# exfinen/zk-toolkit

Hardware: AMD Instinct MI355X
Metric: G1 MSM scalar-muls/sec at 2^20 bases per GPU (BLS12-381) (higher is better)
Workload: dtype u32 limbs (384-bit Montgomery integer)

## Files before the change

### zk-toolkit_amd/csrc/zkt_api.cpp

```cpp
#include <hip/hip_runtime.h>
#include <mutex>
#include <vector>
#include <cstring>
#include <cstdio>
#include <cstdlib>
#include "../../include/zkt.h"
#include "zkt_internal.h"
#include "zkt_constants.h"
#include "host_abi.h"
static_assert(ZKT_G1_PARTIAL_WORDS == 3 * zkt::FqC::N && ZKT_G2_PARTIAL_WORDS == 6 * zkt::FqC::N && ZKT_SECP_PARTIAL_WORDS == 3 * zkt::SpC::N,
              "include/zkt.h partial sizes follow the internal limb layout");

using namespace zkt;

namespace {

struct Ctx {
  bool ready = false;
  int device = -1;
  hipStream_t stream = nullptr;
  unsigned long long* d_err = nullptr;
  uint8_t* arena = nullptr; size_t arena_bytes = 0;
  uint32_t* d_small = nullptr;
  std::mutex mu;
};
Ctx g;
thread_local size_t t_err_index = 0;
thread_local float t_kernel_ms = 0.f;
thread_local const char* t_kernel_name = "";

int ensure_ready() {
  if (!g.ready) return ZKT_ERR_DEVICE;
  return hipSetDevice(g.device) == hipSuccess ? ZKT_OK : ZKT_ERR_DEVICE;
}

int arena_reserve(size_t bytes) {
  if (bytes <= g.arena_bytes) return ZKT_OK;
  if (g.arena) { HIPCHK(hipFree(g.arena)); g.arena = nullptr; g.arena_bytes = 0; }
  size_t want = bytes + (bytes >> 2) + (1 << 20);
  HIPCHK(hipMalloc((void**)&g.arena, want));
  g.arena_bytes = want;
  return ZKT_OK;
}
struct Carver {
  uint8_t* p; size_t off = 0;
  explicit Carver(uint8_t* base) : p(base) {}
  template <class T> T* take(size_t bytes) { off = (off + 255) & ~size_t(255); T* r = (T*)(p + off); off += bytes; return r; }
};
size_t padded(size_t b) { return (b + 255) & ~size_t(255); }

int reset_err(hipStream_t s) {
  unsigned long long v = NO_ERR;
  HIPCHK(hipMemcpyAsync(g.d_err, &v, sizeof(v), hipMemcpyHostToDevice, s));
  return ZKT_OK;
}
int fetch_err(hipStream_t s, int code_if_set) {
  unsigned long long v = NO_ERR;
  HIPCHK(hipMemcpyAsync(&v, g.d_err, sizeof(v), hipMemcpyDeviceToHost, s));
  HIPCHK(hipStreamSynchronize(s));
  if (v != NO_ERR) { t_err_index = (size_t)v; return code_if_set; }
  return ZKT_OK;
}

template <class Launch>
int staged_raw(const void* a, size_t a_total, const void* b, size_t b_total, void* out, size_t out_total, int err_code, Launch launch) {
  if (ensure_ready() != ZKT_OK) return ZKT_ERR_DEVICE;
  if (!a || !out || (b_total && !b)) return ZKT_ERR_SHAPE;
  std::lock_guard<std::mutex> lk(g.mu);
  HIPCHK(hipSetDevice(g.device));
  int rc = arena_reserve(padded(a_total) + padded(b_total) + padded(out_total) + 1024);
  if (rc) return rc;
  Carver cv(g.arena);
  uint32_t* da = cv.take<uint32_t>(a_total);
  uint32_t* db = b_total ? cv.take<uint32_t>(b_total) : nullptr;
  uint32_t* dout = cv.take<uint32_t>(out_total);
  HIPCHK(hipMemcpyAsync(da, a, a_total, hipMemcpyHostToDevice, g.stream));
  if (db) HIPCHK(hipMemcpyAsync(db, b, b_total, hipMemcpyHostToDevice, g.stream));
  if ((rc = reset_err(g.stream))) return rc;
  HIPCHK(launch(da, db, dout, g.stream));
  HIPCHK(hipMemcpyAsync(out, dout, out_total, hipMemcpyDeviceToHost, g.stream));
  return fetch_err(g.stream, err_code);
}
template <class Launch>
int staged(const void* a, size_t a_bytes, const void* b, size_t b_bytes, void* out, size_t out_bytes, size_t n, int err_code, Launch launch) {
  if (ensure_ready() != ZKT_OK) return ZKT_ERR_DEVICE;
  if (n == 0) return ZKT_OK;
  return staged_raw(a, a_bytes * n, b, b_bytes * n, out, out_bytes * n, err_code, launch);
}

size_t field_bytes(int field) { return field == F_FQ ? 48 : 32; }
int fp_batch(int field, int op, const uint64_t* a, const uint64_t* b, uint64_t* out, size_t n) {
  const size_t w = field_bytes(field);
  const bool binary = op == OP_ADD || op == OP_SUB || op == OP_MUL;
  return staged(a, w, binary ? b : nullptr, binary ? w : 0, out, w, n, ZKT_ERR_INV_ZERO,
                [&](uint32_t* da, uint32_t* db, uint32_t* dout, hipStream_t s) { return launch_fp_op(field, op, da, db, dout, n, g.d_err, s); });
}
int fp_pow_batch(int field, const uint64_t* a, const uint64_t* exps, size_t exp_limbs, int exp_shared, uint64_t* out, size_t n) {
  if (exp_limbs == 0 || exp_limbs > 64) return ZKT_ERR_SHAPE;
  if (n == 0) return ensure_ready();
  const size_t w = field_bytes(field);
  return staged_raw(a, w * n, exps, exp_limbs * 8 * (exp_shared ? 1 : n), out, w * n, ZKT_ERR_SHAPE,
                    [&](uint32_t* da, uint32_t* db, uint32_t* dout, hipStream_t s) { return launch_fp_pow(field, da, db, (int)exp_limbs * 2, exp_shared != 0, dout, n, s); });
}
int fp_pow_seq(int field, const uint64_t* base, size_t n, uint64_t* out, bool repeat) {
  if (n == 0) return ensure_ready();
  const size_t w = field_bytes(field);
  return staged_raw(base, w, nullptr, 0, out, w * n, ZKT_ERR_SHAPE,
                    [&](uint32_t* da, uint32_t*, uint32_t* dout, hipStream_t s) { return launch_fp_pow_seq(field, da, dout, n, repeat, s); });
}
int fp_sum(int field, const uint64_t* a, size_t n, uint64_t* out) {
  if (ensure_ready() != ZKT_OK) return ZKT_ERR_DEVICE;
  if (n == 0 || !a || !out) return ZKT_ERR_SHAPE;
  const size_t w = field_bytes(field);
  std::lock_guard<std::mutex> lk(g.mu);
  HIPCHK(hipSetDevice(g.device));
  int rc = arena_reserve(padded(w * n) + padded(w * (1 + fp_sum_scratch_elems())) + 1024);
  if (rc) return rc;
  Carver cv(g.arena);
  uint32_t* da = cv.take<uint32_t>(w * n); uint32_t* dout = cv.take<uint32_t>(w * (1 + fp_sum_scratch_elems()));
  HIPCHK(hipMemcpyAsync(da, a, w * n, hipMemcpyHostToDevice, g.stream));
  HIPCHK(launch_fp_sum(field, da, n, dout, dout + w / 4, g.stream));
  HIPCHK(hipMemcpyAsync(out, dout, w, hipMemcpyDeviceToHost, g.stream));
  HIPCHK(hipStreamSynchronize(g.stream));
  return ZKT_OK;
}
int fp_scale(int field, const uint64_t* a, const uint64_t* k, uint64_t* out, size_t n) {
  if (n == 0) return ZKT_ERR_SHAPE;
  const size_t w = field_bytes(field);
  return staged_raw(a, w * n, k, w, out, w * n, ZKT_ERR_SHAPE,
                    [&](uint32_t* da, uint32_t* db, uint32_t* dout, hipStream_t s) { return launch_fp_scale(field, da, db, dout, n, s); });
}
int tower_batch(int deg, int op, const uint64_t* a, const uint64_t* b, uint64_t* out, size_t n) {
  const size_t w = (size_t)deg * 48;
  const bool binary = op == T_ADD || op == T_SUB || op == T_MUL;
  return staged(a, w, binary ? b : nullptr, binary ? w : 0, out, w, n, ZKT_ERR_INV_ZERO,
                [&](uint32_t* da, uint32_t* db, uint32_t* dout, hipStream_t s) { return launch_tower_op(deg, op, da, db, dout, n, g.d_err, s); });
}

}

static constexpr int MSM_SLOTS = 8;
struct MsmSlot {
  hipEvent_t e_in = nullptr, e_sorted = nullptr, e_acc0 = nullptr, e_acc1 = nullptr, e_done = nullptr;
  void* workspace = nullptr;
  uint32_t* d_result_jac = nullptr;
  uint32_t* d_out_abi = nullptr;
  uint8_t* h_out = nullptr;
  bool busy = false;
  static constexpr int NGRAPH = 4;
  hipGraphExec_t gexec[NGRAPH] = {}; const void* gkey[NGRAPH] = {}; unsigned gnext = 0; bool timed = false;
};
struct zkt_bases_impl {
  size_t n = 0;
  int grp = G_G1;
  MsmPlan plan{};
  uint32_t* table = nullptr;
  uint8_t* inf = nullptr;
  static constexpr int GROUP_TAILS = 4;
  static constexpr int NTAIL = 8;
  hipStream_t s_sort = nullptr, s_acc = nullptr, s_tail[NTAIL] = {};
  bool own_streams = true, acc_owned = false, grouped = false; int tail_base = 0, tail_span = 0;
  MsmSlot slot[MSM_SLOTS];
  std::mutex mu;
};
struct zkt_g1_bases : zkt_bases_impl {};
struct zkt_g2_bases : zkt_bases_impl {};
struct zkt_secp_bases : zkt_bases_impl {};
static size_t grp_coord_bytes(int grp) { return 4 * (grp == G_G1 ? zkt::FqC::N : grp == G_G2 ? 2 * zkt::FqC::N : zkt::SpC::N); }
static int streams_ready(zkt_bases_impl* h) {
  if (h->grouped || !h->own_streams || (h->s_acc && h->s_sort && h->s_tail[zkt_bases_impl::NTAIL - 1])) return ZKT_OK;
  int lo = 0, hi = 0;
  HIPCHK(hipDeviceGetStreamPriorityRange(&lo, &hi));
  if (!h->s_sort) HIPCHK(hipStreamCreateWithPriority(&h->s_sort, hipStreamNonBlocking, hi));
  if (!h->s_acc) HIPCHK(hipStreamCreateWithPriority(&h->s_acc, hipStreamNonBlocking, lo));
  for (int k = 0; k < zkt_bases_impl::NTAIL; ++k) if (!h->s_tail[k]) HIPCHK(hipStreamCreateWithPriority(&h->s_tail[k], hipStreamNonBlocking, hi));
  return ZKT_OK;
}
static bool debug_poison() { static const bool on = [] { const char* e = getenv("ZKT_DEBUG_POISON"); return e && *e == '1'; }(); return on; }
static bool msm_graphs() { static const bool on = [] { const char* e = getenv("ZKT_MSM_GRAPH"); return !(e && *e == '0'); }(); return on; }
static int slot_ready(zkt_bases_impl* h, int k) {
  int rc = streams_ready(h); if (rc) return rc;
  MsmSlot& S = h->slot[k];
  if (S.workspace) return ZKT_OK;
  HIPCHK(hipEventCreateWithFlags(&S.e_in, hipEventDisableTiming)); HIPCHK(hipEventCreateWithFlags(&S.e_sorted, hipEventDisableTiming));
  HIPCHK(hipEventCreate(&S.e_acc0)); HIPCHK(hipEventCreate(&S.e_acc1)); HIPCHK(hipEventCreateWithFlags(&S.e_done, hipEventDisableTiming));
  HIPCHK(hipMalloc(&S.workspace, h->plan.ws_bytes));
  if (debug_poison()) { HIPCHK(hipMemset(S.workspace, 0xA5, h->plan.ws_bytes)); HIPCHK(hipDeviceSynchronize()); }
  HIPCHK(hipMalloc((void**)&S.d_result_jac, 3 * grp_coord_bytes(h->grp)));
  HIPCHK(hipMalloc((void**)&S.d_out_abi, abi_pt_bytes(h->grp)));
  HIPCHK(hipHostMalloc((void**)&S.h_out, abi_pt_bytes(h->grp), hipHostMallocDefault));
  return ZKT_OK;
}

int zkt_internal_ready() { return ensure_ready(); }
hipStream_t zkt_internal_stream() { return g.stream; }
int zkt_internal_device() { return g.device; }
void zkt_internal_set_error_index(size_t i) { t_err_index = i; }

extern "C" {

int zkt_version(void) { return 1; }
const char* zkt_strerror(int s) {
  switch (s) {
    case ZKT_OK: return "ok";
    case ZKT_ERR_INV_ZERO: return "Cannot find inverse of zero";
    case ZKT_ERR_INFINITY: return "pairing argument is the point at infinity";
    case ZKT_ERR_SHAPE: return "bad size, null pointer or non-canonical input";
    case ZKT_ERR_DEVICE: return "no HIP device / HIP error / zkt_init not called";
  }
  return "unknown";
}
size_t zkt_last_error_index(void) { return t_err_index; }
float zkt_last_kernel_ms(void) { return t_kernel_ms; }
const char* zkt_last_kernel_name(void) { return t_kernel_name; }

int zkt_init(int device) {
  std::lock_guard<std::mutex> lk(g.mu);
  if (g.ready) return ZKT_OK;
  int count = 0;
  if (hipGetDeviceCount(&count) != hipSuccess || count == 0) { fprintf(stderr, "[zkt] no HIP device: this library has no CPU path\n"); return ZKT_ERR_DEVICE; }
  if (device < 0) { if (hipGetDevice(&device) != hipSuccess) return ZKT_ERR_DEVICE; }
  if (device >= count) return ZKT_ERR_DEVICE;
  HIPCHK(hipSetDevice(device));
  g.device = device;
  HIPCHK(hipStreamCreateWithFlags(&g.stream, hipStreamNonBlocking));
  HIPCHK(hipMalloc((void**)&g.d_err, 64));
  HIPCHK(hipMalloc((void**)&g.d_small, 4096));
  g.ready = true;
  return ZKT_OK;
}
static void tate_events_release();
void zkt_shutdown(void) {
  if (g.ready) (void)hipSetDevice(g.device);
  zkt_comm_finalize();
  zkt_internal_clear_caches();
  std::lock_guard<std::mutex> lk(g.mu);
  if (!g.ready) return;
  (void)hipSetDevice(g.device);
  group_release_device_state();
  pairing_release_device_state();
  tate_events_release();
  if (g.arena) (void)hipFree(g.arena);
  if (g.d_err) (void)hipFree(g.d_err);
  if (g.d_small) (void)hipFree(g.d_small);
  if (g.stream) (void)hipStreamDestroy(g.stream);
  g.ready = false; g.device = -1; g.stream = nullptr; g.d_err = nullptr; g.d_small = nullptr; g.arena = nullptr; g.arena_bytes = 0;
}

#define FP_BIN(name, field, op) int name(const uint64_t* a, const uint64_t* b, uint64_t* out, size_t n) { return fp_batch(field, op, a, b, out, n); }
#define FP_UN(name, field, op) int name(const uint64_t* a, uint64_t* out, size_t n) { return fp_batch(field, op, a, nullptr, out, n); }
#define FP_FIELD_API(P, F)                                                                                       \
  FP_BIN(zkt_##P##_add_batch, F, OP_ADD) FP_BIN(zkt_##P##_sub_batch, F, OP_SUB) FP_BIN(zkt_##P##_mul_batch, F, OP_MUL) \
  FP_UN(zkt_##P##_sqr_batch, F, OP_SQR) FP_UN(zkt_##P##_neg_batch, F, OP_NEG) FP_UN(zkt_##P##_inv_batch, F, OP_INV)     \
  FP_UN(zkt_##P##_cube_batch, F, OP_CUBE)                                                                        \
  int zkt_##P##_pow_batch(const uint64_t* a, const uint64_t* exps, size_t exp_limbs, int exp_shared, uint64_t* out, size_t n) { \
    return fp_pow_batch(F, a, exps, exp_limbs, exp_shared, out, n); }                                            \
  int zkt_##P##_sum(const uint64_t* a, size_t n, uint64_t* out) { return fp_sum(F, a, n, out); }                   \
  int zkt_##P##_scale_batch(const uint64_t* a, const uint64_t* k, uint64_t* out, size_t n) { return fp_scale(F, a, k, out, n); } \
  int zkt_##P##_pow_seq(const uint64_t* base, size_t n, uint64_t* out) { return fp_pow_seq(F, base, n, out, false); }  \
  int zkt_##P##_repeat(const uint64_t* base, size_t n, uint64_t* out) { return fp_pow_seq(F, base, n, out, true); }
FP_FIELD_API(fq, F_FQ) FP_FIELD_API(fr, F_FR) FP_FIELD_API(sp, F_SP) FP_FIELD_API(sn, F_SN)

#define TW_BIN(name, deg, op) int name(const uint64_t* a, const uint64_t* b, uint64_t* out, size_t n) { return tower_batch(deg, op, a, b, out, n); }
#define TW_UN(name, deg, op) int name(const uint64_t* a, uint64_t* out, size_t n) { return tower_batch(deg, op, a, nullptr, out, n); }
TW_BIN(zkt_fq2_add_batch, 2, T_ADD) TW_BIN(zkt_fq2_sub_batch, 2, T_SUB) TW_BIN(zkt_fq2_mul_batch, 2, T_MUL)
TW_UN(zkt_fq2_inv_batch, 2, T_INV) TW_UN(zkt_fq2_neg_batch, 2, T_NEG) TW_UN(zkt_fq2_reduce_batch, 2, T_REDUCE)
TW_BIN(zkt_fq6_add_batch, 6, T_ADD) TW_BIN(zkt_fq6_sub_batch, 6, T_SUB) TW_BIN(zkt_fq6_mul_batch, 6, T_MUL)
TW_UN(zkt_fq6_inv_batch, 6, T_INV) TW_UN(zkt_fq6_neg_batch, 6, T_NEG) TW_UN(zkt_fq6_reduce_batch, 6, T_REDUCE)
TW_BIN(zkt_fq12_add_batch, 12, T_ADD) TW_BIN(zkt_fq12_sub_batch, 12, T_SUB) TW_BIN(zkt_fq12_mul_batch, 12, T_MUL)
TW_UN(zkt_fq12_inv_batch, 12, T_INV) TW_UN(zkt_fq12_neg_batch, 12, T_NEG)

int zkt_fq12_pow_batch(const uint64_t* a, const uint32_t* e, size_t nl, uint64_t* out, size_t n) {
  if (!e || nl == 0 || nl > 4096) return ZKT_ERR_SHAPE;
  if (ensure_ready() != ZKT_OK) return ZKT_ERR_DEVICE;
  if (n == 0) return ZKT_OK;
  if (!a || !out) return ZKT_ERR_SHAPE;
  std::lock_guard<std::mutex> lk(g.mu);
  HIPCHK(hipSetDevice(g.device));
  int rc = arena_reserve(padded(576 * n) * 2 + padded(nl * 4) + 1024);
  if (rc) return rc;
  Carver cv(g.arena);
  uint32_t* da = cv.take<uint32_t>(576 * n); uint32_t* dout = cv.take<uint32_t>(576 * n); uint32_t* de = cv.take<uint32_t>(nl * 4);
  HIPCHK(hipMemcpyAsync(da, a, 576 * n, hipMemcpyHostToDevice, g.stream));
  HIPCHK(hipMemcpyAsync(de, e, nl * 4, hipMemcpyHostToDevice, g.stream));
  HIPCHK(launch_fq12_pow(da, de, (int)nl, dout, n, g.stream));
  HIPCHK(hipMemcpyAsync(out, dout, 576 * n, hipMemcpyDeviceToHost, g.stream));
  HIPCHK(hipStreamSynchronize(g.stream));
  return ZKT_OK;
}

int zkt_selftest_fq_program(uint64_t seed0, int steps, const uint64_t* in, uint64_t* out, int32_t* violations, size_t count) {
  if (ensure_ready() != ZKT_OK) return ZKT_ERR_DEVICE;
  if (count == 0) return ZKT_OK;
  if (!in || !out || !violations || steps < 0) return ZKT_ERR_SHAPE;
  std::lock_guard<std::mutex> lk(g.mu);
  HIPCHK(hipSetDevice(g.device));
  const size_t eb = 4 * 48;
  int rc = arena_reserve(padded(eb * count) * 2 + padded(4 * count) + 1024);
  if (rc) return rc;
  Carver cv(g.arena);
  uint32_t* din = cv.take<uint32_t>(eb * count); uint32_t* dout = cv.take<uint32_t>(eb * count); int* dbad = (int*)cv.take<uint32_t>(4 * count);
  HIPCHK(hipMemcpyAsync(din, in, eb * count, hipMemcpyHostToDevice, g.stream));
  HIPCHK(launch_selftest_fq_program(seed0, steps, din, dout, dbad, count, g.stream));
  HIPCHK(hipMemcpyAsync(out, dout, eb * count, hipMemcpyDeviceToHost, g.stream));
  HIPCHK(hipMemcpyAsync(violations, dbad, 4 * count, hipMemcpyDeviceToHost, g.stream));
  HIPCHK(hipStreamSynchronize(g.stream));
  return ZKT_OK;
}

int zkt_debug_dfq12_op(int op, const uint64_t* a, const uint64_t* b, uint64_t* out, size_t n) {
  if (op < 0 || op > 6) return ZKT_ERR_SHAPE;
  return staged(a, 576, op == 0 ? b : nullptr, op == 0 ? 576 : 0, out, 576, n, ZKT_ERR_SHAPE,
                [&](uint32_t* da, uint32_t* db, uint32_t* dout, hipStream_t s) { return launch_dfq12_op(op, da, db, dout, n, s); });
}

static int group_add(int grp, const void* a, const void* b, void* out, size_t n) {
  size_t w = abi_pt_bytes(grp);
  return staged(a, w, b, w, out, w, n, ZKT_ERR_SHAPE,
                [&](uint32_t* da, uint32_t* db, uint32_t* dout, hipStream_t s) { return launch_group_add(grp, da, db, dout, n, s); });
}
static int group_neg(int grp, const void* a, void* out, size_t n) {
  size_t w = abi_pt_bytes(grp);
  return staged(a, w, nullptr, 0, out, w, n, ZKT_ERR_SHAPE,
                [&](uint32_t* da, uint32_t*, uint32_t* dout, hipStream_t s) { return launch_group_neg(grp, da, dout, n, s); });
}
static int group_mul(int grp, const void* pts, const uint64_t* scalars, int limbs, void* out, size_t n) {
  if (limbs < 1 || limbs > 6) return ZKT_ERR_SHAPE;
  size_t w = abi_pt_bytes(grp);
  return staged(pts, w, scalars, (size_t)limbs * 8, out, w, n, ZKT_ERR_SHAPE,
                [&](uint32_t* da, uint32_t* db, uint32_t* dout, hipStream_t s) { return launch_group_mul(grp, da, db, limbs * 2, dout, n, s); });
}
static int group_sum(int grp, const void* pts, size_t n, void* out) {
  if (ensure_ready() != ZKT_OK) return ZKT_ERR_DEVICE;
  const size_t w = abi_pt_bytes(grp);
  if (!out || (n && !pts)) return ZKT_ERR_SHAPE;
  if (n == 0) { memset(out, 0, w); ((uint32_t*)out)[w / 4 - 2] = 1; return ZKT_OK; }
  std::lock_guard<std::mutex> lk(g.mu);
  HIPCHK(hipSetDevice(g.device));
  int rc = arena_reserve(padded(w * (n + 1)) + 1024);
  if (rc) return rc;
  Carver cv(g.arena);
  uint32_t* da = cv.take<uint32_t>(w * (n + 1));
  HIPCHK(hipMemcpyAsync(da, pts, w * n, hipMemcpyHostToDevice, g.stream));
  if (n == 1) {
    std::vector<uint8_t> inf(w, 0); ((uint32_t*)inf.data())[w / 4 - 2] = 1;
    HIPCHK(hipMemcpyAsync((uint8_t*)da + w, inf.data(), w, hipMemcpyHostToDevice, g.stream));
    HIPCHK(hipStreamSynchronize(g.stream));
  }
  HIPCHK(launch_group_sum_inplace(grp, da, n == 1 ? 2 : n, g.stream));
  HIPCHK(hipMemcpyAsync(out, da, w, hipMemcpyDeviceToHost, g.stream));
  HIPCHK(hipStreamSynchronize(g.stream));
  return ZKT_OK;
}
static int group_scale(int grp, const void* pts, const uint64_t* k, int limbs, void* out, size_t n) {
  if (limbs < 1 || limbs > 6) return ZKT_ERR_SHAPE;
  if (n == 0) return ensure_ready();
  size_t w = abi_pt_bytes(grp);
  return staged_raw(pts, w * n, k, (size_t)limbs * 8, out, w * n, ZKT_ERR_SHAPE,
                    [&](uint32_t* da, uint32_t* db, uint32_t* dout, hipStream_t s) { return launch_group_mul(grp, da, db, limbs * 2, dout, n, s, false, true); });
}
int zkt_g1_sum(const zkt_g1_affine* p, size_t n, zkt_g1_affine* o) { return group_sum(G_G1, p, n, o); }
int zkt_g2_sum(const zkt_g2_affine* p, size_t n, zkt_g2_affine* o) { return group_sum(G_G2, p, n, o); }
int zkt_secp_sum(const zkt_secp_affine* p, size_t n, zkt_secp_affine* o) { return group_sum(G_SECP, p, n, o); }
int zkt_g1_scale_batch(const zkt_g1_affine* p, const uint64_t* k, int l, zkt_g1_affine* o, size_t n) { return group_scale(G_G1, p, k, l, o, n); }
int zkt_g2_scale_batch(const zkt_g2_affine* p, const uint64_t* k, int l, zkt_g2_affine* o, size_t n) { return group_scale(G_G2, p, k, l, o, n); }
int zkt_secp_scale_batch(const zkt_secp_affine* p, const uint64_t* k, int l, zkt_secp_affine* o, size_t n) { return group_scale(G_SECP, p, k, l, o, n); }
int zkt_g1_add_batch(const zkt_g1_affine* a, const zkt_g1_affine* b, zkt_g1_affine* o, size_t n) { return group_add(G_G1, a, b, o, n); }
int zkt_g2_add_batch(const zkt_g2_affine* a, const zkt_g2_affine* b, zkt_g2_affine* o, size_t n) { return group_add(G_G2, a, b, o, n); }
int zkt_secp_add_batch(const zkt_secp_affine* a, const zkt_secp_affine* b, zkt_secp_affine* o, size_t n) { return group_add(G_SECP, a, b, o, n); }
int zkt_g1_neg_batch(const zkt_g1_affine* a, zkt_g1_affine* o, size_t n) { return group_neg(G_G1, a, o, n); }
int zkt_g2_neg_batch(const zkt_g2_affine* a, zkt_g2_affine* o, size_t n) { return group_neg(G_G2, a, o, n); }
int zkt_g1_mul_batch(const zkt_g1_affine* p, const uint64_t* k, int l, zkt_g1_affine* o, size_t n) { return group_mul(G_G1, p, k, l, o, n); }
int zkt_g2_mul_batch(const zkt_g2_affine* p, const uint64_t* k, int l, zkt_g2_affine* o, size_t n) { return group_mul(G_G2, p, k, l, o, n); }
int zkt_secp_mul_batch(const zkt_secp_affine* p, const uint64_t* k, int l, zkt_secp_affine* o, size_t n) { return group_mul(G_SECP, p, k, l, o, n); }

static int group_pred(int grp, int pred, const void* pts, uint32_t* out, size_t n) {
  uint32_t order[8];
  for (int i = 0; i < 8; ++i) order[i] = grp == G_SECP ? SnC::mod32(i) : FrC::mod32(i);
  return staged(pts, abi_pt_bytes(grp), nullptr, 0, out, 4, n, ZKT_ERR_SHAPE,
                [&](uint32_t* da, uint32_t*, uint32_t* dout, hipStream_t s) -> hipError_t {
                  uint32_t* d_order = g.d_small;
                  hipError_t e = hipMemcpyAsync(d_order, order, 32, hipMemcpyHostToDevice, s);
                  if (e != hipSuccess) return e;
                  return launch_group_pred(grp, pred, da, d_order, 8, dout, n, s);
                });
}
int zkt_g1_is_on_curve_batch(const zkt_g1_affine* p, uint32_t* out, size_t n) { return group_pred(G_G1, 0, p, out, n); }
int zkt_g2_is_on_curve_batch(const zkt_g2_affine* p, uint32_t* out, size_t n) { return group_pred(G_G2, 0, p, out, n); }
int zkt_secp_is_on_curve_batch(const zkt_secp_affine* p, uint32_t* out, size_t n) { return group_pred(G_SECP, 0, p, out, n); }
int zkt_g1_in_subgroup_batch(const zkt_g1_affine* p, uint32_t* out, size_t n) { return group_pred(G_G1, 1, p, out, n); }
int zkt_g2_in_subgroup_batch(const zkt_g2_affine* p, uint32_t* out, size_t n) { return group_pred(G_G2, 1, p, out, n); }
int zkt_secp_in_subgroup_batch(const zkt_secp_affine* p, uint32_t* out, size_t n) { return group_pred(G_SECP, 1, p, out, n); }
void zkt_g1_generator(zkt_g1_affine* out) { *out = G1_GEN; }
void zkt_g2_generator(zkt_g2_affine* out) { *out = G2_GEN; }
void zkt_secp_generator(zkt_secp_affine* out) { *out = SECP_GEN; }

int zkt_tate_batch(const zkt_g1_affine* g1, const zkt_g2_affine* g2, uint64_t* out, size_t n) {
  return staged(g1, sizeof(zkt_g1_affine), g2, sizeof(zkt_g2_affine), out, 576, n, ZKT_ERR_INFINITY,
                [&](uint32_t* da, uint32_t* db, uint32_t* dout, hipStream_t s) { return launch_tate(da, db, dout, n, g.d_err, s); });
}
static int miller_exact(int which, const zkt_g1_affine* g1, const zkt_g2_affine* g2, uint64_t* out, size_t n) {
  return staged(g1, sizeof(zkt_g1_affine), g2, sizeof(zkt_g2_affine), out, 576, n, ZKT_ERR_INFINITY,
                [&](uint32_t* da, uint32_t* db, uint32_t* dout, hipStream_t s) { return launch_miller_exact(which, da, db, dout, n, g.d_err, s); });
}
int zkt_miller_g1g2_batch(const zkt_g1_affine* g1, const zkt_g2_affine* g2, uint64_t* out, size_t n) { return miller_exact(0, g1, g2, out, n); }
int zkt_miller_g2g1_batch(const zkt_g2_affine* g2, const zkt_g1_affine* g1, uint64_t* out, size_t n) { return miller_exact(1, g1, g2, out, n); }
int zkt_weil_batch(const zkt_g1_affine* g1, const zkt_g2_affine* g2, uint64_t* out, size_t n) { return miller_exact(2, g1, g2, out, n); }
int zkt_gt_eq(const uint64_t* a, const uint64_t* b) {
  if (!a || !b) return -ZKT_ERR_SHAPE;
  return memcmp(a, b, 576) == 0 ? 1 : 0;
}

int zkt_fq_mul_batch_dev(const uint64_t* a, const uint64_t* b, uint64_t* out, size_t n, void* stream) {
  if (ensure_ready() != ZKT_OK) return ZKT_ERR_DEVICE;
  HIPCHK(launch_fp_op(F_FQ, OP_MUL, (const uint32_t*)a, (const uint32_t*)b, (uint32_t*)out, n, g.d_err, (hipStream_t)stream));
  return ZKT_OK;
}
int zkt_g1_mul_batch_dev(const zkt_g1_affine* p, const uint64_t* k, int limbs, zkt_g1_affine* out, size_t n, void* stream) {
  if (ensure_ready() != ZKT_OK) return ZKT_ERR_DEVICE;
  if (limbs < 1 || limbs > 6) return ZKT_ERR_SHAPE;
  HIPCHK(launch_group_mul(G_G1, (const uint32_t*)p, (const uint32_t*)k, limbs * 2, (uint32_t*)out, n, (hipStream_t)stream));
  return ZKT_OK;
}
int zkt_g2_mul_batch_dev(const zkt_g2_affine* p, const uint64_t* k, int limbs, zkt_g2_affine* out, size_t n, void* stream) {
  if (ensure_ready() != ZKT_OK) return ZKT_ERR_DEVICE;
  if (limbs < 1 || limbs > 6) return ZKT_ERR_SHAPE;
  HIPCHK(launch_group_mul(G_G2, (const uint32_t*)p, (const uint32_t*)k, limbs * 2, (uint32_t*)out, n, (hipStream_t)stream));
  return ZKT_OK;
}
static hipEvent_t g_tate_ev[3] = {nullptr, nullptr, nullptr};
static int tate_events() {
  if (g_tate_ev[0]) return ZKT_OK;
  hipEvent_t e[3] = {nullptr, nullptr, nullptr};
  if (hipEventCreateWithFlags(&e[0], hipEventDisableTiming) != hipSuccess || hipEventCreate(&e[1]) != hipSuccess || hipEventCreate(&e[2]) != hipSuccess) {
    for (hipEvent_t x : e) if (x) (void)hipEventDestroy(x);
    (void)hipGetLastError(); return ZKT_ERR_DEVICE;
  }
  for (int i = 0; i < 3; ++i) g_tate_ev[i] = e[i];
  return ZKT_OK;
}
static void tate_events_release() { for (hipEvent_t& x : g_tate_ev) { if (x) (void)hipEventDestroy(x); x = nullptr; } }
int zkt_tate_batch_dev(const zkt_g1_affine* g1, const zkt_g2_affine* g2, uint64_t* out, size_t n, void* stream) {
  if (ensure_ready() != ZKT_OK) return ZKT_ERR_DEVICE;
  std::lock_guard<std::mutex> lk(g.mu);
  hipStream_t s = g.stream;
  int rc = tate_events(); if (rc) return rc;
  HIPCHK(hipEventRecord(g_tate_ev[0], (hipStream_t)stream));
  HIPCHK(hipStreamWaitEvent(s, g_tate_ev[0], 0));
  rc = reset_err(s); if (rc) return rc;
  HIPCHK(hipEventRecord(g_tate_ev[1], s));
  HIPCHK(launch_tate((const uint32_t*)g1, (const uint32_t*)g2, (uint32_t*)out, n, g.d_err, s));
  HIPCHK(hipEventRecord(g_tate_ev[2], s));
  rc = fetch_err(s, ZKT_ERR_INFINITY);
  HIPCHK(hipEventElapsedTime(&t_kernel_ms, g_tate_ev[1], g_tate_ev[2])); t_kernel_name = "k_tate";
  return rc;
}

static int bases_build(zkt_bases_impl* h, const uint32_t* dev_abi, hipStream_t s) {
  const size_t n = h->n;
  h->plan = msm_plan(n, h->grp);
  const size_t tot = (size_t)h->plan.nwin * (n ? n : 1);
  HIPCHK(hipMalloc((void**)&h->table, tot * 2 * grp_coord_bytes(h->grp)));
  HIPCHK(hipMalloc((void**)&h->inf, tot));
  HIPCHK(launch_msm_to_kernel_layout(h->grp, dev_abi, h->table, h->inf, n, s));
  uint32_t* tmp = nullptr;
  if (h->plan.nwin > 1) HIPCHK(hipMalloc((void**)&tmp, (size_t)(h->plan.nwin - 1) * (n ? n : 1) * 2 * grp_coord_bytes(h->grp)));
  hipError_t e = launch_msm_precompute(h->grp, h->table, h->inf, n, h->plan.c, h->plan.nwin, tmp, s);
  if (e == hipSuccess) e = hipStreamSynchronize(s);
  if (tmp) hipFree(tmp);
  HIPCHK(e);
  return ZKT_OK;
}
static void bases_free(zkt_bases_impl* h) {
  if (!h) return;
  if (h->table) hipFree(h->table);
  if (h->inf) hipFree(h->inf);
  if (h->own_streams) {
    for (hipStream_t st : {h->s_sort, h->s_acc}) if (st) { hipStreamSynchronize(st); hipStreamDestroy(st); }
    for (hipStream_t st : h->s_tail) if (st) { hipStreamSynchronize(st); hipStreamDestroy(st); }
  } else {
    for (hipStream_t st : {h->s_sort, h->s_acc}) if (st) hipStreamSynchronize(st);
    for (hipStream_t st : h->s_tail) if (st) hipStreamSynchronize(st);
    if (h->acc_owned && h->s_acc) hipStreamDestroy(h->s_acc);
  }
  for (MsmSlot& S : h->slot) {
    for (hipEvent_t ev : {S.e_in, S.e_sorted, S.e_acc0, S.e_acc1, S.e_done}) if (ev) hipEventDestroy(ev);
    for (hipGraphExec_t& ge : S.gexec) if (ge) { (void)hipGraphExecDestroy(ge); ge = nullptr; }
    if (S.workspace) hipFree(S.workspace); if (S.d_result_jac) hipFree(S.d_result_jac); if (S.d_out_abi) hipFree(S.d_out_abi);
    if (S.h_out) hipHostFree(S.h_out);
  }
  delete h;
}
static int bases_from_device(int grp, const void* dev_bases, size_t n, void* stream, zkt_bases_impl** out) {
  if (ensure_ready() != ZKT_OK) return ZKT_ERR_DEVICE;
  if (!out || (n && !dev_bases) || n >= (size_t(1) << 26)) return ZKT_ERR_SHAPE;
  zkt_bases_impl* h = new zkt_bases_impl(); h->n = n; h->grp = grp;
  int rc = bases_build(h, (const uint32_t*)dev_bases, (hipStream_t)stream);
  if (rc) { bases_free(h); return rc; }
  *out = h; return ZKT_OK;
}
static int bases_upload(int grp, const void* host, size_t n, zkt_bases_impl** out) {
  if (ensure_ready() != ZKT_OK) return ZKT_ERR_DEVICE;
  if (!out || (n && !host)) return ZKT_ERR_SHAPE;
  HIPCHK(hipSetDevice(g.device));
  uint32_t* tmp = nullptr;
  HIPCHK(hipMalloc((void**)&tmp, (n ? n : 1) * abi_pt_bytes(grp)));
  if (n) HIPCHK(hipMemcpy(tmp, host, n * abi_pt_bytes(grp), hipMemcpyHostToDevice));
  int rc = bases_from_device(grp, tmp, n, g.stream, out);
  hipFree(tmp);
  return rc;
}
static hipStream_t slot_tail_stream(zkt_bases_impl* h, int slot) {
  if (h->grouped) return h->s_tail[(h->tail_base + slot % h->tail_span) % zkt_bases_impl::GROUP_TAILS];
  const bool small = h->n < (size_t(1) << 19);
  return h->s_tail[small ? slot % zkt_bases_impl::NTAIL : slot % 2];
}
static int msm_submit_locked(zkt_bases_impl* h, const uint64_t* dev_scalars, size_t n, void* stream, int slot) {
  if (n != h->n || (n && !dev_scalars) || slot < 0 || slot >= MSM_SLOTS) return ZKT_ERR_SHAPE;
  if (h->slot[slot].busy) return ZKT_ERR_SHAPE;
  int rc = slot_ready(h, slot); if (rc) return rc;
  MsmSlot& S = h->slot[slot];
  HIPCHK(hipEventRecord(S.e_in, (hipStream_t)stream));
  const bool small = h->n < (size_t(1) << 19);
  hipStream_t st = slot_tail_stream(h, slot);
  hipStream_t ss = small ? st : h->s_sort;
  HIPCHK(hipStreamWaitEvent(ss, S.e_in, 0));
  if (small && msm_graphs()) {
    int hit = -1;
    for (int k = 0; k < MsmSlot::NGRAPH; ++k) if (S.gexec[k] && S.gkey[k] == (const void*)dev_scalars) hit = k;
    if (hit < 0) {
      hit = (int)(S.gnext++ % MsmSlot::NGRAPH);
      if (S.gexec[hit]) { (void)hipGraphExecDestroy(S.gexec[hit]); S.gexec[hit] = nullptr; }
      hipGraph_t graph = nullptr;
      HIPCHK(hipStreamBeginCapture(st, hipStreamCaptureModeRelaxed));
      hipError_t e = launch_msm_sort(h->plan, h->inf, (const uint32_t*)dev_scalars, S.workspace, st);
      if (e == hipSuccess) e = launch_msm_accumulate(h->plan, h->table, S.workspace, st);
      if (e == hipSuccess) e = launch_msm_reduce(h->plan, S.workspace, S.d_result_jac, S.d_out_abi, st);
      const hipError_t e2 = hipStreamEndCapture(st, &graph);
      if (e != hipSuccess || e2 != hipSuccess || !graph) { if (graph) (void)hipGraphDestroy(graph); HIPCHK(e != hipSuccess ? e : (e2 != hipSuccess ? e2 : hipErrorUnknown)); }
      e = hipGraphInstantiate(&S.gexec[hit], graph, nullptr, nullptr, 0);
      (void)hipGraphDestroy(graph);
      if (e != hipSuccess) { S.gexec[hit] = nullptr; HIPCHK(e); }
      S.gkey[hit] = (const void*)dev_scalars;
    }
    HIPCHK(hipGraphLaunch(S.gexec[hit], st));
    HIPCHK(hipMemcpyAsync(S.h_out, S.d_out_abi, abi_pt_bytes(h->grp), hipMemcpyDeviceToHost, st));
    HIPCHK(hipEventRecord(S.e_done, st));
    S.timed = false; S.busy = true;
    return ZKT_OK;
  }
  S.timed = true;
  HIPCHK(launch_msm_sort(h->plan, h->inf, (const uint32_t*)dev_scalars, S.workspace, ss));
  HIPCHK(hipEventRecord(S.e_sorted, ss));
  hipStream_t sa = small ? st : h->s_acc;
  HIPCHK(hipStreamWaitEvent(sa, S.e_sorted, 0));
  HIPCHK(hipEventRecord(S.e_acc0, sa));
  HIPCHK(launch_msm_accumulate(h->plan, h->table, S.workspace, sa));
  HIPCHK(hipEventRecord(S.e_acc1, sa));
  HIPCHK(hipStreamWaitEvent(st, S.e_acc1, 0));
  HIPCHK(launch_msm_reduce(h->plan, S.workspace, S.d_result_jac, S.d_out_abi, st));
  HIPCHK(hipMemcpyAsync(S.h_out, S.d_out_abi, abi_pt_bytes(h->grp), hipMemcpyDeviceToHost, st));
  HIPCHK(hipEventRecord(S.e_done, st));
  S.busy = true;
  return ZKT_OK;
}
static int msm_collect_locked(zkt_bases_impl* h, int slot, void* out, uint32_t* dev_partial_jac) {
  if (slot < 0 || slot >= MSM_SLOTS || !h->slot[slot].busy) return ZKT_ERR_SHAPE;
  MsmSlot& S = h->slot[slot];
  HIPCHK(hipEventSynchronize(S.e_done));
  if (dev_partial_jac) {
    hipStream_t st = slot_tail_stream(h, slot);
    HIPCHK(hipMemcpyAsync(dev_partial_jac, S.d_result_jac, 3 * grp_coord_bytes(h->grp), hipMemcpyDeviceToDevice, st));
    HIPCHK(hipStreamSynchronize(st));
  }
  if (out) memcpy(out, S.h_out, abi_pt_bytes(h->grp));
  float ms = 0.f;
  if (S.timed && hipEventElapsedTime(&ms, S.e_acc0, S.e_acc1) == hipSuccess) { t_kernel_ms = ms; t_kernel_name = "k_accumulate"; }
  else { t_kernel_ms = 0.f; t_kernel_name = "msm_graph"; }
  S.busy = false;
  return ZKT_OK;
}
static int msm_submit(zkt_bases_impl* h, const uint64_t* dev_scalars, size_t n, void* stream, int slot) {
  if (ensure_ready() != ZKT_OK) return ZKT_ERR_DEVICE;
  if (!h) return ZKT_ERR_SHAPE;
  std::lock_guard<std::mutex> lk(h->mu);
  return msm_submit_locked(h, dev_scalars, n, stream, slot);
}
static int msm_collect(zkt_bases_impl* h, int slot, void* out, uint32_t* dev_partial_jac) {
  if (ensure_ready() != ZKT_OK) return ZKT_ERR_DEVICE;
  if (!h) return ZKT_ERR_SHAPE;
  std::lock_guard<std::mutex> lk(h->mu);
  return msm_collect_locked(h, slot, out, dev_partial_jac);
}
static int msm_dev(zkt_bases_impl* h, const uint64_t* dev_scalars, size_t n, void* stream, void* out, uint32_t* dev_partial_jac) {
  if (ensure_ready() != ZKT_OK) return ZKT_ERR_DEVICE;
  if (!h || (!out && !dev_partial_jac)) return ZKT_ERR_SHAPE;
  std::lock_guard<std::mutex> lk(h->mu);
  int rc = msm_submit_locked(h, dev_scalars, n, stream, 0);
  if (rc) return rc;
  return msm_collect_locked(h, 0, out, dev_partial_jac);
}
int zkt_internal_bases_share_streams(void* dst_, void* src_, int share_acc, int tail_base, int tail_span) {
  zkt_bases_impl *dst = (zkt_bases_impl*)dst_, *src = (zkt_bases_impl*)src_;
  if (!dst || !src || tail_span < 1 || tail_base < 0) return ZKT_ERR_SHAPE;
  constexpr int GROUP_TAILS = zkt_bases_impl::GROUP_TAILS;
  if (tail_base >= GROUP_TAILS || tail_span > GROUP_TAILS) return ZKT_ERR_SHAPE;
  int lo = 0, hi = 0; HIPCHK(hipDeviceGetStreamPriorityRange(&lo, &hi));
  {
    std::lock_guard<std::mutex> lk(src->mu);
    if (!src->grouped) {
      if (src->s_sort || src->s_acc) return ZKT_ERR_SHAPE;
      HIPCHK(hipStreamCreateWithPriority(&src->s_sort, hipStreamNonBlocking, hi)); HIPCHK(hipStreamCreateWithPriority(&src->s_acc, hipStreamNonBlocking, lo));
      for (int k = 0; k < GROUP_TAILS; ++k) HIPCHK(hipStreamCreateWithPriority(&src->s_tail[k], hipStreamNonBlocking, hi));
      src->grouped = true; src->tail_base = 0; src->tail_span = 2;
    }
  }
  std::lock_guard<std::mutex> lk(dst->mu);
  if (dst->s_sort || dst->s_acc) return ZKT_ERR_SHAPE;
  dst->own_streams = false; dst->grouped = true; dst->s_sort = src->s_sort;
  for (int k = 0; k < GROUP_TAILS; ++k) dst->s_tail[k] = src->s_tail[k];
  dst->tail_base = tail_base; dst->tail_span = tail_span;
  if (share_acc) dst->s_acc = src->s_acc;
  else { HIPCHK(hipStreamCreateWithPriority(&dst->s_acc, hipStreamNonBlocking, lo)); dst->acc_owned = true; }
  return ZKT_OK;
}
int zkt_internal_jac_sum(int grp, const uint32_t* dev_partials, size_t count, size_t stride_words, hipStream_t s, void* out) {
  if (!dev_partials || !out || count == 0) return ZKT_ERR_SHAPE;
  std::lock_guard<std::mutex> lk(g.mu);
  HIPCHK(launch_msm_jac_sum_to_affine(grp, dev_partials, count, stride_words, g.d_small, s));
  HIPCHK(hipMemcpyAsync(out, g.d_small, abi_pt_bytes(grp), hipMemcpyDeviceToHost, s));
  HIPCHK(hipStreamSynchronize(s));
  return ZKT_OK;
}
static int jac_sum_dev(int grp, const uint32_t* dev_partials, size_t count, void* stream, void* out) {
  if (ensure_ready() != ZKT_OK) return ZKT_ERR_DEVICE;
  return zkt_internal_jac_sum(grp, dev_partials, count, 3 * grp_coord_bytes(grp) / 4, (hipStream_t)stream, out);
}
static int msm_host(int grp, const void* bases, const uint64_t* scalars, size_t n, void* out) {
  if (ensure_ready() != ZKT_OK) return ZKT_ERR_DEVICE;
  if (!out || (n && (!bases || !scalars)) || n >= (size_t(1) << 26)) return ZKT_ERR_SHAPE;
  if (n == 0) { memset(out, 0, abi_pt_bytes(grp)); ((uint32_t*)out)[abi_pt_bytes(grp) / 4 - 2] = 1; return ZKT_OK; }
  const MsmPlan plan = msm_plan_direct(n, grp);
  const size_t ptb = abi_pt_bytes(grp), cb = grp_coord_bytes(grp);
  uint8_t* blob = nullptr;
  const size_t o_abi = 0, o_sc = padded(n * ptb), o_tab = o_sc + padded(n * 32), o_inf = o_tab + padded(n * 2 * cb), o_jac = o_inf + padded(n),
               o_out = o_jac + padded(4 * cb), o_ws = o_out + padded(ptb), total = o_ws + plan.ws_bytes;
  HIPCHK(hipMalloc((void**)&blob, total));
  if (debug_poison()) { HIPCHK(hipMemset(blob, 0xA5, total)); HIPCHK(hipDeviceSynchronize()); }
  std::lock_guard<std::mutex> lk(g.mu);
  hipStream_t s = g.stream;
  int rc = ZKT_OK;
  auto fail = [&](hipError_t e) { if (e != hipSuccess) { fprintf(stderr, "[zkt] HIP error %s in one-shot MSM\n", hipGetErrorString(e)); rc = ZKT_ERR_DEVICE; } return e != hipSuccess; };
  if (!fail(hipMemcpyAsync(blob + o_abi, bases, n * ptb, hipMemcpyHostToDevice, s)) && !fail(hipMemcpyAsync(blob + o_sc, scalars, n * 32, hipMemcpyHostToDevice, s)) &&
      !fail(launch_msm_to_kernel_layout(grp, (const uint32_t*)(blob + o_abi), (uint32_t*)(blob + o_tab), blob + o_inf, n, s)) &&
      !fail(launch_msm_sort(plan, blob + o_inf, (const uint32_t*)(blob + o_sc), blob + o_ws, s)) &&
      !fail(launch_msm_accumulate(plan, (const uint32_t*)(blob + o_tab), blob + o_ws, s)) &&
      !fail(launch_msm_reduce(plan, blob + o_ws, (uint32_t*)(blob + o_jac), (uint32_t*)(blob + o_out), s)) &&
      !fail(hipMemcpyAsync(out, blob + o_out, ptb, hipMemcpyDeviceToHost, s)))
    fail(hipStreamSynchronize(s));
  else hipStreamSynchronize(s);
  hipFree(blob);
  return rc;
}

#define ZKT_BASES_API(NAME, GRP, PT)                                                                                             \
  int zkt_##NAME##_bases_from_device(const PT* dev, size_t n, void* stream, zkt_##NAME##_bases** out) {                          \
    return bases_from_device(GRP, dev, n, stream, (zkt_bases_impl**)out); }                                                     \
  int zkt_##NAME##_bases_upload(const PT* host, size_t n, zkt_##NAME##_bases** out) { return bases_upload(GRP, host, n, (zkt_bases_impl**)out); } \
  size_t zkt_##NAME##_bases_len(const zkt_##NAME##_bases* b) { return b ? b->n : 0; }                                             \
  void zkt_##NAME##_bases_free(zkt_##NAME##_bases* b) { bases_free(b); }                                                          \
  int zkt_##NAME##_msm_submit(zkt_##NAME##_bases* b, const uint64_t* k, size_t n, void* stream, int slot) { return msm_submit(b, k, n, stream, slot); } \
  int zkt_##NAME##_msm_collect(zkt_##NAME##_bases* b, int slot, PT* out, uint32_t* partial) { return msm_collect(b, slot, out, partial); } \
  int zkt_##NAME##_msm_dev(const zkt_##NAME##_bases* b, const uint64_t* k, size_t n, void* stream, PT* out, uint32_t* partial) { \
    return msm_dev(const_cast<zkt_##NAME##_bases*>(b), k, n, stream, out, partial); }                                              \
  int zkt_##NAME##_jac_sum_dev(const uint32_t* partials, size_t count, void* stream, PT* out) { return jac_sum_dev(GRP, partials, count, stream, out); } \
  int zkt_##NAME##_msm(const PT* bases, const uint64_t* scalars, size_t n, PT* out) { return msm_host(GRP, bases, scalars, n, out); }
ZKT_BASES_API(g1, G_G1, zkt_g1_affine)
ZKT_BASES_API(g2, G_G2, zkt_g2_affine)
ZKT_BASES_API(secp, G_SECP, zkt_secp_affine)
size_t zkt_g1_msm_workspace_bytes(size_t n) { MsmPlan p = msm_plan(n, G_G1); return p.ws_bytes + (size_t)p.nwin * n * 97; }

}
```

### zk-toolkit_amd/csrc/zkt_internal.h

```cpp
#pragma once
#include <hip/hip_runtime.h>
#include <stdint.h>
#include <stddef.h>

namespace zkt {

enum FieldId { F_FQ = 0, F_FR = 1, F_SP = 2, F_SN = 3 };
enum FpOp { OP_ADD = 0, OP_SUB = 1, OP_MUL = 2, OP_SQR = 3, OP_NEG = 4, OP_INV = 5, OP_CUBE = 6 };
enum TowerOp { T_ADD = 0, T_SUB = 1, T_MUL = 2, T_INV = 3, T_NEG = 4, T_REDUCE = 5 };
enum GroupId { G_G1 = 0, G_G2 = 1, G_SECP = 2 };

static constexpr unsigned long long NO_ERR = ~0ull;

static inline unsigned grid_blocks(size_t n, unsigned tpb = 256) { return (unsigned)((n + tpb - 1) / tpb); }

hipError_t launch_fp_op(int field, int op, const uint32_t* a, const uint32_t* b, uint32_t* out, size_t n,
                        unsigned long long* err, hipStream_t s);
hipError_t launch_fp_pow(int field, const uint32_t* a, const uint32_t* e, int e_words, bool shared, uint32_t* out, size_t n, hipStream_t s);
hipError_t launch_fp_pow_seq(int field, const uint32_t* base, uint32_t* out, size_t n, bool repeat, hipStream_t s);
size_t fp_sum_scratch_elems();
hipError_t launch_fp_sum(int field, const uint32_t* a, size_t n, uint32_t* out, uint32_t* parts, hipStream_t s);
hipError_t launch_fp_scale(int field, const uint32_t* a, const uint32_t* k, uint32_t* out, size_t n, hipStream_t s);
hipError_t launch_selftest_fq_program(unsigned long long seed0, int steps, const uint32_t* in4, uint32_t* out4, int* bad, size_t count, hipStream_t s);
hipError_t launch_tower_op(int deg, int op, const uint32_t* a, const uint32_t* b, uint32_t* out, size_t n,
                           unsigned long long* err, hipStream_t s);
hipError_t launch_fq12_pow(const uint32_t* a, const uint32_t* exp_dev, int exp_nlimbs, uint32_t* out, size_t n, hipStream_t s);
hipError_t launch_group_add(int grp, const uint32_t* a, const uint32_t* b, uint32_t* out, size_t n, hipStream_t s);
hipError_t launch_group_neg(int grp, const uint32_t* a, uint32_t* out, size_t n, hipStream_t s);
hipError_t launch_group_mul(int grp, const uint32_t* pts, const uint32_t* scalars, int scalar_words, uint32_t* out, size_t n, hipStream_t s, bool fixed_base = false, bool fixed_scalar = false);
struct G1Fits { const uint32_t* pts[4]; uint32_t stride[4]; };
hipError_t launch_g1_fits(const G1Fits& f, int K, uint32_t* out, size_t n, hipStream_t s);

hipError_t launch_group_pred(int grp, int pred, const uint32_t* pts, const uint32_t* order, int order_words, uint32_t* out, size_t n, hipStream_t s);
hipError_t launch_group_sum_inplace(int grp, uint32_t* pts, size_t n, hipStream_t s);
struct MulSeg { const uint32_t* pts; const uint32_t* k; uint32_t* out; uint32_t count, pt_stride, k_stride; };
struct MulSegs { MulSeg s[16]; int n; };
hipError_t launch_group_mul_segs(int grp, const MulSegs& segs, int scalar_words, hipStream_t s);
struct ScalarOp { int op; const uint32_t* a; const uint32_t* b; uint32_t* out; };
struct ScalarOps { ScalarOp o[48]; int n; };
hipError_t launch_scalar_ops(int field, const ScalarOps& ops, unsigned long long* err, hipStream_t s);
struct PointSums { const uint32_t* in[12][4]; int cnt[12]; uint32_t* out[12]; int n; };
hipError_t launch_point_sums(int grp, const PointSums& p, hipStream_t s);
struct FixedMul { const uint32_t* table; const uint32_t* k; uint32_t* out; };
struct FixedMuls { FixedMul m[16]; int n; };
struct FixedTables { const uint32_t* point[12]; uint32_t* table[12]; int n; };
hipError_t launch_fixed_tables(int grp, const FixedTables& t, hipStream_t s);
hipError_t launch_generator_mul(int grp, const uint32_t* gen_abi, const uint32_t* k, uint32_t* out, size_t n, hipStream_t s);
hipError_t launch_fixed_muls(int grp, const FixedMuls& f, hipStream_t s);
hipError_t launch_fixed_muls_batch(int grp, const uint32_t* tables, const uint32_t* k, uint32_t* out, size_t n, int n_pts, hipStream_t s);
hipError_t launch_miller_exact(int which, const uint32_t* g1, const uint32_t* g2, uint32_t* out, size_t n, unsigned long long* err, hipStream_t s);
hipError_t launch_groth16_verify(const uint32_t* A, const uint32_t* B, const uint32_t* C, const uint32_t* uvw_stmt, const uint32_t* stmt, int n_stmt,
                                 const uint32_t* gamma, const uint32_t* delta, const uint32_t* alpha_beta, uint32_t* ok, size_t n,
                                 unsigned long long* err, hipStream_t s, const uint32_t* ate_key = nullptr);
static constexpr size_t ATE_KEY_WORDS = 2 * (size_t)68 * 84 + 144 + 1;
hipError_t launch_ate_key_prep(const uint32_t* alpha, const uint32_t* beta, const uint32_t* gamma, const uint32_t* delta, const uint32_t* uvw_stmt, int n_stmt,
                               uint32_t* key, hipStream_t s);
size_t stmt_wide_table_words(int n_pts);
hipError_t launch_stmt_wide_tables(const uint32_t* tab16, int n_pts, uint32_t* tables, hipStream_t s);
hipError_t launch_stmt_sums_wide(const uint32_t* tables, const uint32_t* stmt, int n_stmt, uint32_t* out, size_t n, hipStream_t s);
void verify_set_fail_closed(int on);
int verify_fail_closed();
size_t dproduct_limit();
hipError_t launch_groth16_verify_small(const uint32_t* A, const uint32_t* B, const uint32_t* C, const uint32_t* uvw_stmt, const uint32_t* stmt_tables, const uint32_t* stmt, int n_stmt,
                                       const uint32_t* gamma, const uint32_t* delta, const uint32_t* alpha_beta, uint32_t* tmp, uint32_t* S, uint32_t* ok, size_t n,
                                       unsigned long long* err, hipStream_t s, const uint32_t* ate_target = nullptr);
struct PairArgs { const uint32_t* g1[4]; const uint32_t* g2[4]; uint32_t s1[4], s2[4]; uint32_t neg[4]; };
hipError_t launch_pairing_product_check(const PairArgs& a, int K, uint32_t* ok, size_t n, unsigned long long* err, hipStream_t s, uint32_t p_trusted = 0);
hipError_t launch_dfq12_op(int op, const uint32_t* a, const uint32_t* b, uint32_t* out, size_t n, hipStream_t s);
hipError_t launch_dtate(const uint32_t* g1, const uint32_t* g2, uint32_t* out, size_t n, unsigned long long* err, uint32_t mark_word, uint32_t mark, hipStream_t s);
hipError_t launch_dproduct(const PairArgs& a, int K, const uint32_t* target, uint32_t* ok, size_t n, unsigned long long* err, hipStream_t s, const uint8_t* kcount = nullptr);
hipError_t launch_dproduct_ate(const PairArgs& a, int K, const uint32_t* target, uint32_t* ok, size_t n, unsigned long long* err, hipStream_t s, const uint8_t* kcount = nullptr);
hipError_t launch_key_ab(const uint32_t* alpha, const uint32_t* beta, uint32_t* out, uint32_t* flag, uint32_t bit, uint32_t* gt, hipStream_t s);
hipError_t launch_ate_guards(const PairArgs& a, int K, uint32_t* flags, size_t n, hipStream_t s, uint32_t p_skip = 0);
hipError_t launch_pairing_product_check_counts(const PairArgs& a, int K, const uint8_t* kcount, uint32_t* ok, size_t n, unsigned long long* err, hipStream_t s);
hipError_t guard_fork(hipStream_t s, hipStream_t* side);
hipError_t guard_join(hipStream_t s, hipStream_t side);
hipError_t launch_short_loop_guards(const PairArgs& a, int K, uint32_t* flags, size_t n, hipStream_t s);
void group_release_device_state();
void pairing_release_device_state();
hipError_t launch_tate(const uint32_t* g1, const uint32_t* g2, uint32_t* out, size_t n, unsigned long long* err, hipStream_t s);

struct MsmPlan {
  size_t n;
  int grp;
  int c;
  int nwin;
  size_t nbuckets;
  size_t ws_bytes;
  int direct;
  size_t half;
  uint32_t chunk;
};
MsmPlan msm_plan(size_t n, int grp);
MsmPlan msm_plan_direct(size_t n, int grp);
hipError_t launch_msm_to_kernel_layout(int grp, const uint32_t* abi_pts, uint32_t* table, uint8_t* base_inf, size_t n, hipStream_t s);
hipError_t launch_msm_precompute(int grp, uint32_t* table, uint8_t* inf, size_t n, int c, int nwin, uint32_t* tmp, hipStream_t s);
hipError_t launch_msm_sort(const MsmPlan& plan, const uint8_t* base_inf, const uint32_t* scalars, void* workspace, hipStream_t s);
hipError_t launch_msm_accumulate(const MsmPlan& plan, const uint32_t* table, void* workspace, hipStream_t s);
hipError_t launch_msm_reduce(const MsmPlan& plan, void* workspace, uint32_t* dev_result_jac, uint32_t* dev_out_abi, hipStream_t s);
hipError_t launch_msm_jac_add(int grp, const uint32_t* a, const uint32_t* b, uint32_t* out, hipStream_t s);
hipError_t launch_msm_jac_sum_to_affine(int grp, const uint32_t* jac_partials, size_t count, size_t stride_words, uint32_t* out_abi_pt, hipStream_t s);

}

hipError_t zkt_launch_accumulate_g2_pair(const uint32_t* table, const uint32_t* entries, const uint32_t* offsets, const void* order, const uint32_t* task_off,
                                         size_t nbuckets, uint32_t* sums, uint32_t* partial, size_t max_tasks, hipStream_t s);

int zkt_internal_ready();
hipStream_t zkt_internal_stream();
void zkt_internal_set_error_index(size_t i);
extern "C" int zkt_internal_bases_share_streams(void* dst, void* src, int share_acc, int tail_base, int tail_span);
extern "C" int zkt_internal_jac_sum(int grp, const uint32_t* dev_partials, size_t count, size_t stride_words, hipStream_t s, void* out);
extern "C" void zkt_internal_clear_caches();
extern "C" void zkt_pinocchio_clear_caches();
```

### zk-toolkit_amd/csrc/zkt_msm.hip

```cpp
#include <cstdlib>
#include "abi.h"
#include "zkt_internal.h"

namespace zkt {

#ifndef ZKT_SIDE_PRIO
#define ZKT_SIDE_PRIO __builtin_amdgcn_s_setprio(3)
#endif
template <class F> struct Coord;
template <class C> struct Coord<PrimeOps<C>> {
  static constexpr int CW = C::N;
  __device__ static Fp<C> ld(const uint32_t* p) { return ld_raw<C>(p); }
  __device__ static void st(uint32_t* p, const Fp<C>& a) { st_raw<C>(p, a); }
};
template <> struct Coord<Fq2Ops> {
  static constexpr int CW = 2 * FqC::N;
  __device__ static Fq2 ld(const uint32_t* p) { Fq2 r; r.c0 = ld_raw<FqC>(p); r.c1 = ld_raw<FqC>(p + FqC::N); return r; }
  __device__ static void st(uint32_t* p, const Fq2& a) { st_raw<FqC>(p, a.c0); st_raw<FqC>(p + FqC::N, a.c1); }
};
template <class F> __device__ inline Xyzz<F> ld_xy(const uint32_t* p) {
  constexpr int CW = Coord<F>::CW; Xyzz<F> r;
  r.X = Coord<F>::ld(p); r.Y = Coord<F>::ld(p + CW); r.ZZ = Coord<F>::ld(p + 2 * CW); r.ZZZ = Coord<F>::ld(p + 3 * CW); return r;
}
template <class F> __device__ inline void st_xy(uint32_t* p, const Xyzz<F>& a) {
  constexpr int CW = Coord<F>::CW;
  Coord<F>::st(p, a.X); Coord<F>::st(p + CW, a.Y); Coord<F>::st(p + 2 * CW, a.ZZ); Coord<F>::st(p + 3 * CW, a.ZZZ);
}
static int coord_words(int grp) { return grp == G_G1 ? FqC::N : grp == G_G2 ? 2 * FqC::N : SpC::N; }
static constexpr int PART_LO = 9, PART_SUB = 1 << PART_LO, PART_TPB = 256, PART_TILE = 4 * PART_TPB, PART_CHUNK = 8192, PART_MAXP = 2048;
struct PartDims { uint32_t P, ntiles, maxblk; };
static PartDims part_dims(size_t n, size_t nbuckets, int nwin) {
  PartDims d; d.P = (uint32_t)((nbuckets + PART_SUB - 1) / PART_SUB); d.ntiles = (uint32_t)((n + PART_TILE - 1) / PART_TILE);
  d.maxblk = d.P + (uint32_t)((size_t)nwin * n / PART_CHUNK) + 1; return d;
}
static size_t part_ws_bytes(size_t n, size_t nbuckets, int nwin) {
  const PartDims d = part_dims(n, nbuckets, nwin);
  return 1024 + (size_t)nwin * n * 8 + 256 + 2 * ((size_t)d.P * d.ntiles + 1) * 4 + ((size_t)d.P + 1) * 4 + ((size_t)d.P * d.ntiles / 2048 + 2) * 4 + 256 + (size_t)d.maxblk * PART_SUB * 4;
}

#if defined(ZKT_MSM_PART_G1)
static constexpr uint32_t MSM_CHUNK_MAX = 128;
static uint32_t pick_chunk(size_t entries, int grp);
MsmPlan msm_plan(size_t n, int grp) {
  MsmPlan p; p.n = n; p.grp = grp;
  const size_t XYW = 4 * (size_t)coord_words(grp);
  int lg = 0; while ((size_t(1) << (lg + 1)) <= (n ? n : 1)) ++lg;
  static const int forced_c = [] { const char* e = getenv("ZKT_MSM_C"); return e ? atoi(e) : 0; }();
  int c = lg >= 19 ? 20 : lg >= 14 ? 16 : lg >= 11 ? 13 : lg == 10 ? 11 : 10;
  if (forced_c) c = forced_c;
  if (c < 4) c = 4;
  if (c > 20) c = 20;
  p.c = c; p.nwin = (256 + 1 + c - 1) / c; p.nbuckets = size_t(1) << (c - 1);
  size_t ent = (size_t)p.nwin * n;
  p.chunk = pick_chunk(ent, grp);
  size_t b = 0;
  b += (p.nbuckets + 1) * 4 * 3;
  b += 2 * ent * 4 + 256;
  b += p.nbuckets * XYW * 4;
  b += (2048 + 64 * 4) * XYW * 4;
  b += (1024 + 3 * 1025) * 4 + 2 * (p.nbuckets + 1) * 4;
  b += (p.nbuckets + ent / p.chunk + 2) * (8 + XYW * 4);
  b += 64 * 64 * XYW * 4 + 1024;
  b += part_ws_bytes(n, p.nbuckets, p.nwin);
  b += 4096;
  p.ws_bytes = b;
  p.direct = 0; p.half = p.nbuckets;
  return p;
}
static uint32_t pick_chunk(size_t entries, int grp) {
  const size_t tasks = grp == G_G2 ? (size_t)65536 : (size_t)196608;
  size_t c = (entries + tasks - 1) / tasks;
  if (c < 8) c = 8;
  if (c > MSM_CHUNK_MAX) c = MSM_CHUNK_MAX;
  return (uint32_t)c;
}
MsmPlan msm_plan_direct(size_t n, int grp) {
  MsmPlan p; p.n = n; p.grp = grp;
  const size_t XYW = 4 * (size_t)coord_words(grp);
  int lg = 0; while ((size_t(1) << (lg + 1)) <= (n ? n : 1)) ++lg;
  int c = lg - 3;
  if (c < 9) c = 9;
  if (c > 16) c = 16;
  p.c = c; p.nwin = (256 + 1 + c - 1) / c; p.half = size_t(1) << (c - 1); p.nbuckets = (size_t)p.nwin * p.half; p.direct = 1;
  size_t ent = (size_t)p.nwin * n;
  p.chunk = pick_chunk(ent, grp);
  size_t b = 0;
  b += (p.nbuckets + 1) * 4 * 3 + 2 * ent * 4 + 256 + p.nbuckets * XYW * 4;
  b += (size_t)p.nwin * (2048 + 64 * 4 + 1) * XYW * 4;
  b += (1024 + 3 * 1025) * 4 + 2 * (p.nbuckets + 1) * 4;
  b += (p.nbuckets + ent / p.chunk + 2) * (8 + XYW * 4);
  b += 64 * 64 * XYW * 4 + 1024;
  b += part_ws_bytes(n, p.nbuckets, p.nwin);
  b += 8192;
  p.ws_bytes = b;
  return p;
}
#endif

template <class F>
__global__ void __launch_bounds__(64) k_to_kernel_layout(const uint32_t* __restrict__ abi, uint32_t* __restrict__ mont,
                                                         uint8_t* __restrict__ inf, size_t n) {
  size_t i = (size_t)blockIdx.x * 64 + threadIdx.x;
  if (i >= n) return;
  constexpr int CW = Coord<F>::CW;
  Aff<F> p = PtIO<F>::ld(abi + i * PtIO<F>::WORDS);
  Coord<F>::st(mont + i * 2 * CW, p.x); Coord<F>::st(mont + i * 2 * CW + CW, p.y);
  inf[i] = p.inf ? 1 : 0;
}
#if defined(ZKT_MSM_PART_G1)
#define MSM_DISPATCH(grp, CALL) switch (grp) { case G_G1: { typedef FqOps F; CALL; } break; default: return hipErrorInvalidValue; }
#define PART(x) x##_g1
#elif defined(ZKT_MSM_PART_SECP)
#define MSM_DISPATCH(grp, CALL) switch (grp) { case G_SECP: { typedef SpOps F; CALL; } break; default: return hipErrorInvalidValue; }
#define PART(x) x##_secp
#else
#define MSM_DISPATCH(grp, CALL) switch (grp) { case G_G2: { typedef Fq2Ops F; CALL; } break; default: return hipErrorInvalidValue; }
#define PART(x) x##_other
#endif
hipError_t PART(launch_msm_to_kernel_layout)(int grp, const uint32_t* abi, uint32_t* mont, uint8_t* inf, size_t n, hipStream_t s) {
  if (n == 0) return hipSuccess;
  MSM_DISPATCH(grp, hipLaunchKernelGGL(k_to_kernel_layout<F>, dim3(grid_blocks(n, 64)), dim3(64), 0, s, abi, mont, inf, n));
  return hipGetLastError();
}

template <class F>
__global__ void __launch_bounds__(64) k_precompute(uint32_t* __restrict__ table, uint8_t* __restrict__ inf, size_t n, int c, int nwin, uint32_t* __restrict__ tmp) {
  size_t i = (size_t)blockIdx.x * 64 + threadIdx.x;
  if (i >= n || nwin < 2) return;
  constexpr int CW = Coord<F>::CW, PW = 2 * CW;
  typedef typename F::E E;
  Aff<F> a; a.x = Coord<F>::ld(table + i * PW); a.y = Coord<F>::ld(table + i * PW + CW); a.inf = inf[i] != 0;
  Jac<F> j = jac_from_aff(a);
  E acc = F::one();
  for (int w = 1; w < nwin; ++w) {
    for (int d = 0; d < c; ++d) j = jac_dbl(j);
    const size_t o = (size_t)w * n + i, t = (size_t)(w - 1) * n + i;
    const bool isinf = jac_is_inf(j);
    const E z = isinf ? F::one() : j.Z;
    Coord<F>::st(table + o * PW, j.X); Coord<F>::st(table + o * PW + CW, j.Y);
    Coord<F>::st(tmp + t * PW, z); Coord<F>::st(tmp + t * PW + CW, acc);
    inf[o] = isinf ? 1 : 0;
    acc = F::mul(acc, z);
  }
  E inv = F::inv(acc);
  for (int w = nwin - 1; w >= 1; --w) {
    const size_t o = (size_t)w * n + i, t = (size_t)(w - 1) * n + i;
    const E z = Coord<F>::ld(tmp + t * PW), pre = Coord<F>::ld(tmp + t * PW + CW);
    const E zi = F::mul(inv, pre);
    inv = F::mul(inv, z);
    const E zi2 = F::sqr(zi);
    E x = F::mul(Coord<F>::ld(table + o * PW), zi2), y = F::mul(Coord<F>::ld(table + o * PW + CW), F::mul(zi2, zi));
    if (inf[o]) { x = F::zero(); y = F::zero(); }
    Coord<F>::st(table + o * PW, x); Coord<F>::st(table + o * PW + CW, y);
  }
}

__device__ inline uint32_t window_bits(const uint32_t* k, int w, int c) {
  int o = w * c, word = o >> 5, sh = o & 31;
  if (word >= 8) return 0;
  uint64_t v = k[word];
  if (word + 1 < 8) v |= (uint64_t)k[word + 1] << 32;
  return (uint32_t)(v >> sh) & ((1u << c) - 1);
}

static constexpr uint32_t NO_SLOT = 0xffffffffu;
template <bool SCATTER>
static __global__ void __launch_bounds__(256) k_digits(const uint32_t* __restrict__ scalars, const uint8_t* __restrict__ inf, size_t n, int c, int nwin, uint32_t win_buckets,
                                                uint32_t* __restrict__ counts, const uint32_t* __restrict__ offsets,
                                                uint32_t* __restrict__ slot, uint32_t* __restrict__ entries) {
  ZKT_SIDE_PRIO;
  size_t i = (size_t)blockIdx.x * 256 + threadIdx.x;
  const bool live = i < n;
  uint32_t k[8] = {0, 0, 0, 0, 0, 0, 0, 0};
  if (live) {
    const uint4* sp = reinterpret_cast<const uint4*>(scalars + i * 8);
    uint4 lo = sp[0], hi = sp[1];
    k[0] = lo.x; k[1] = lo.y; k[2] = lo.z; k[3] = lo.w; k[4] = hi.x; k[5] = hi.y; k[6] = hi.z; k[7] = hi.w;
  }
  const uint32_t half = 1u << (c - 1);
  const unsigned lane = threadIdx.x & 63;
  const unsigned long long lt_mask = (1ull << lane) - 1ull;
  uint32_t carry = 0;
  for (int w = 0; w < nwin; ++w) {
    uint32_t raw = window_bits(k, w, c) + carry;
    uint32_t neg = raw > half;
    uint32_t mag = neg ? (1u << c) - raw : raw;
    carry = neg;
    size_t src = win_buckets ? i : (size_t)w * n + i;
    const uint32_t b = mag - 1 + (uint32_t)w * win_buckets;
    if (SCATTER) {
      if (live) { const uint32_t pos = slot[(size_t)w * n + i]; if (pos != NO_SLOT) entries[offsets[b] + pos] = (uint32_t)src | (neg << 31); }
      continue;
    }
    bool todo = live && mag != 0 && !inf[live ? src : 0];
    uint32_t pos = NO_SLOT;
    for (int round = 0; round < 2; ++round) {
      unsigned long long act = __ballot(todo);
      if (act == 0) break;
      int leader = __ffsll((long long)act) - 1;
      uint32_t lb = __shfl(b, leader);
      unsigned long long same = __ballot(todo && b == lb);
      int cnt = __popcll(same);
      if (cnt < 4) break;
      uint32_t base = 0;
      if ((int)lane == leader) base = atomicAdd(&counts[lb], (uint32_t)cnt);
      base = __shfl(base, leader);
      if (todo && b == lb) { pos = base + (uint32_t)__popcll(same & lt_mask); todo = false; }
    }
    if (todo) pos = atomicAdd(&counts[b], 1u);
    if (live) slot[(size_t)w * n + i] = pos;
  }
}

static constexpr int SCAN_TPB = 256, SCAN_ITEMS = 8, SCAN_TILE = SCAN_TPB * SCAN_ITEMS;
__device__ inline uint32_t block_excl_scan_256(uint32_t v, uint32_t* lds , uint32_t& total) {
  const int t = threadIdx.x;
  lds[t] = v; __syncthreads();
  for (int d = 1; d < 256; d <<= 1) {
    uint32_t x = t >= d ? lds[t - d] : 0; __syncthreads();
    lds[t] += x; __syncthreads();
  }
  total = lds[255];
  uint32_t excl = t ? lds[t - 1] : 0;
  __syncthreads();
  return excl;
}
static __global__ void __launch_bounds__(256) k_scan_sums(const uint32_t* __restrict__ in, size_t m, uint32_t* __restrict__ blocksum) {
  ZKT_SIDE_PRIO;
  __shared__ uint32_t lds[256];
  size_t base = (size_t)blockIdx.x * SCAN_TILE + (size_t)threadIdx.x * SCAN_ITEMS;
  uint32_t s = 0;
#pragma unroll
  for (int k = 0; k < SCAN_ITEMS; ++k) if (base + k < m) s += in[base + k];
  uint32_t tot; (void)block_excl_scan_256(s, lds, tot);
  if (threadIdx.x == 0) blocksum[blockIdx.x] = tot;
}
static __global__ void __launch_bounds__(256) k_scan_top(uint32_t* __restrict__ blocksum, int nblk, uint32_t* __restrict__ grand_total) {
  ZKT_SIDE_PRIO;
  __shared__ uint32_t lds[256];
  uint32_t run = 0;
  for (int base = 0; base < nblk; base += 256) {
    int i = base + threadIdx.x;
    uint32_t v = i < nblk ? blocksum[i] : 0, tot;
    uint32_t ex = block_excl_scan_256(v, lds, tot);
    if (i < nblk) blocksum[i] = run + ex;
    run += tot;
  }
  if (threadIdx.x == 0) *grand_total = run;
}
static __global__ void __launch_bounds__(256) k_scan_final(const uint32_t* __restrict__ in, size_t m, const uint32_t* __restrict__ blocksum,
                                                    uint32_t* __restrict__ out) {
  ZKT_SIDE_PRIO;
  __shared__ uint32_t lds[256];
  size_t base = (size_t)blockIdx.x * SCAN_TILE + (size_t)threadIdx.x * SCAN_ITEMS;
  uint32_t v[SCAN_ITEMS], s = 0;
#pragma unroll
  for (int k = 0; k < SCAN_ITEMS; ++k) { v[k] = base + k < m ? in[base + k] : 0; s += v[k]; }
  uint32_t tot; uint32_t run = block_excl_scan_256(s, lds, tot) + blocksum[blockIdx.x];
#pragma unroll
  for (int k = 0; k < SCAN_ITEMS; ++k) { if (base + k < m) out[base + k] = run; run += v[k]; }
}
static void launch_scan(const uint32_t* in, uint32_t* out, size_t m, uint32_t* scratch, hipStream_t s) {
  int nblk = (int)((m + SCAN_TILE - 1) / SCAN_TILE);
  hipLaunchKernelGGL(k_scan_sums, dim3(nblk), dim3(256), 0, s, in, m, scratch);
  hipLaunchKernelGGL(k_scan_top, dim3(1), dim3(256), 0, s, scratch, nblk, out + m);
  hipLaunchKernelGGL(k_scan_final, dim3(nblk), dim3(256), 0, s, in, m, (const uint32_t*)scratch, out);
}

template <bool SCATTER>
static __global__ void __launch_bounds__(PART_TPB) k_part_tiles(const uint32_t* __restrict__ scalars, const uint8_t* __restrict__ inf, size_t n, int c, int nwin, uint32_t win_buckets,
                                                    uint32_t P, uint32_t ntiles, uint32_t* __restrict__ tilehist, const uint32_t* __restrict__ tileoff,
                                                    uint2* __restrict__ rec) {
  ZKT_SIDE_PRIO;
  __shared__ uint32_t h[PART_MAXP];
  for (uint32_t p = threadIdx.x; p < P; p += PART_TPB) h[p] = SCATTER ? tileoff[(size_t)p * ntiles + blockIdx.x] : 0u;
  __syncthreads();
  const uint32_t half = 1u << (c - 1);
  for (int j = 0; j < PART_TILE / PART_TPB; j += 2) {
    const size_t i0 = (size_t)blockIdx.x * PART_TILE + j * PART_TPB + threadIdx.x, i1 = i0 + PART_TPB;
    const bool v0 = i0 < n, v1 = i1 < n;
    uint32_t k0[8] = {}, k1[8] = {};
    if (v0) { const uint4* sp = reinterpret_cast<const uint4*>(scalars + i0 * 8); const uint4 lo = sp[0], hi = sp[1];
      k0[0] = lo.x; k0[1] = lo.y; k0[2] = lo.z; k0[3] = lo.w; k0[4] = hi.x; k0[5] = hi.y; k0[6] = hi.z; k0[7] = hi.w; }
    if (v1) { const uint4* sp = reinterpret_cast<const uint4*>(scalars + i1 * 8); const uint4 lo = sp[0], hi = sp[1];
      k1[0] = lo.x; k1[1] = lo.y; k1[2] = lo.z; k1[3] = lo.w; k1[4] = hi.x; k1[5] = hi.y; k1[6] = hi.z; k1[7] = hi.w; }
    uint32_t carry0 = 0, carry1 = 0;
    for (int w = 0; w < nwin; ++w) {
      const uint32_t raw0 = window_bits(k0, w, c) + carry0, raw1 = window_bits(k1, w, c) + carry1;
      const uint32_t neg0 = raw0 > half, neg1 = raw1 > half;
      const uint32_t mag0 = neg0 ? (1u << c) - raw0 : raw0, mag1 = neg1 ? (1u << c) - raw1 : raw1;
      carry0 = neg0; carry1 = neg1;
      const size_t src0 = win_buckets ? i0 : (size_t)w * n + i0, src1 = win_buckets ? i1 : (size_t)w * n + i1;
      const bool a0 = v0 && mag0 != 0 && !inf[src0], a1 = v1 && mag1 != 0 && !inf[src1];
      const uint32_t b0 = mag0 - 1 + (uint32_t)w * win_buckets, b1 = mag1 - 1 + (uint32_t)w * win_buckets;
      uint32_t pos0 = 0, pos1 = 0;
      if (a0) pos0 = atomicAdd(&h[b0 >> PART_LO], 1u);
      if (a1) pos1 = atomicAdd(&h[b1 >> PART_LO], 1u);
      if (SCATTER) {
        if (a0) rec[pos0] = make_uint2((uint32_t)src0 | (neg0 << 31), b0 & (PART_SUB - 1));
        if (a1) rec[pos1] = make_uint2((uint32_t)src1 | (neg1 << 31), b1 & (PART_SUB - 1));
      }
    }
  }
  if (!SCATTER) {
    __syncthreads();
    for (uint32_t p = threadIdx.x; p < P; p += PART_TPB) tilehist[(size_t)p * ntiles + blockIdx.x] = h[p];
  }
}
static __global__ void __launch_bounds__(256) k_part_blocks(const uint32_t* __restrict__ tileoff, uint32_t P, uint32_t ntiles, uint32_t* __restrict__ blkoff) {
  ZKT_SIDE_PRIO;
  __shared__ uint32_t lds[256];
  constexpr int ITEMS = PART_MAXP / 256;
  uint32_t v[ITEMS], sum = 0;
#pragma unroll
  for (int k = 0; k < ITEMS; ++k) {
    const uint32_t p = threadIdx.x * ITEMS + k;
    uint32_t cnt = 0;
    if (p < P) { const uint32_t size = tileoff[(size_t)(p + 1) * ntiles] - tileoff[(size_t)p * ntiles]; cnt = (size + PART_CHUNK - 1) / PART_CHUNK; }
    v[k] = cnt; sum += cnt;
  }
  uint32_t tot; uint32_t run = block_excl_scan_256(sum, lds, tot);
#pragma unroll
  for (int k = 0; k < ITEMS; ++k) { const uint32_t p = threadIdx.x * ITEMS + k; if (p < P) blkoff[p] = run; run += v[k]; }
  if (threadIdx.x == 0) blkoff[P] = tot;
}
__device__ inline uint32_t part_of_block(const uint32_t* __restrict__ blkoff, uint32_t P, uint32_t blk) {
  uint32_t lo = 0, hi = P;
  while (hi - lo > 1) { const uint32_t mid = (lo + hi) >> 1; if (blkoff[mid] <= blk) lo = mid; else hi = mid; }
  return lo;
}
template <bool PLACE>
static __global__ void __launch_bounds__(256) k_part_chunks(const uint32_t* __restrict__ tileoff, uint32_t P, uint32_t ntiles, const uint32_t* __restrict__ blkoff,
                                                     const uint2* __restrict__ rec, uint32_t* __restrict__ subhist,
                                                     const uint32_t* __restrict__ offsets, size_t nbuckets, uint32_t* __restrict__ entries) {
  ZKT_SIDE_PRIO;
  __shared__ uint32_t h[PART_SUB];
  const uint32_t blk = blockIdx.x;
  if (blk >= blkoff[P]) return;
  const uint32_t p = part_of_block(blkoff, P, blk), chunk = blk - blkoff[p];
  const uint32_t pbeg = tileoff[(size_t)p * ntiles], pend = tileoff[(size_t)(p + 1) * ntiles];
  const uint32_t beg = pbeg + chunk * PART_CHUNK, end = beg + PART_CHUNK < pend ? beg + PART_CHUNK : pend;
  for (int t = threadIdx.x; t < PART_SUB; t += 256) {
    const size_t b = (size_t)p * PART_SUB + t;
    h[t] = PLACE ? (b < nbuckets ? offsets[b] + subhist[(size_t)blk * PART_SUB + t] : 0u) : 0u;
  }
  __syncthreads();
  uint32_t r = beg + threadIdx.x;
  for (; r + 3 * 256 < end; r += 4 * 256) {
    const uint2 r0 = rec[r], r1 = rec[r + 256], r2 = rec[r + 512], r3 = rec[r + 768];
    const uint32_t p0 = atomicAdd(&h[r0.y], 1u), p1 = atomicAdd(&h[r1.y], 1u), p2 = atomicAdd(&h[r2.y], 1u), p3 = atomicAdd(&h[r3.y], 1u);
    if (PLACE) { entries[p0] = r0.x; entries[p1] = r1.x; entries[p2] = r2.x; entries[p3] = r3.x; }
  }
  for (; r < end; r += 256) {
    const uint2 rr = rec[r];
    const uint32_t pos = atomicAdd(&h[rr.y], 1u);
    if (PLACE) entries[pos] = rr.x;
  }
  if (!PLACE) {
    __syncthreads();
    for (int t = threadIdx.x; t < PART_SUB; t += 256) subhist[(size_t)blk * PART_SUB + t] = h[t];
  }
}
static __global__ void __launch_bounds__(PART_SUB) k_part_offsets(const uint32_t* __restrict__ tileoff, uint32_t P, uint32_t ntiles, const uint32_t* __restrict__ blkoff,
                                                           uint32_t* __restrict__ subhist, size_t nbuckets, uint32_t* __restrict__ counts, uint32_t* __restrict__ offsets) {
  ZKT_SIDE_PRIO;
  __shared__ uint32_t sc[PART_SUB];
  const uint32_t p = blockIdx.x, t = threadIdx.x;
  uint32_t run = 0;
  for (uint32_t cblk = blkoff[p]; cblk < blkoff[p + 1]; ++cblk) { const uint32_t v = subhist[(size_t)cblk * PART_SUB + t]; subhist[(size_t)cblk * PART_SUB + t] = run; run += v; }
  sc[t] = run; __syncthreads();
  for (int d = 1; d < PART_SUB; d <<= 1) { const uint32_t x = t >= (uint32_t)d ? sc[t - d] : 0u; __syncthreads(); sc[t] += x; __syncthreads(); }
  const size_t b = (size_t)p * PART_SUB + t;
  if (b < nbuckets) { counts[b] = run; offsets[b] = tileoff[(size_t)p * ntiles] + sc[t] - run; }
  if (p == P - 1 && t == 0) offsets[nbuckets] = tileoff[(size_t)P * ntiles];
}

static constexpr uint32_t CHUNK = 128;
static constexpr int SIZE_BINS = CHUNK + 1;
__device__ inline uint32_t ntasks_of(uint32_t c, uint32_t chunk) { return c <= chunk ? 1u : (c + chunk - 1) / chunk; }
__device__ inline uint32_t task_size_of(uint32_t c, uint32_t nt) { return (c + nt - 1) / nt; }
static __global__ void __launch_bounds__(256) k_task_count(const uint32_t* __restrict__ counts, size_t m, uint32_t chunk, uint32_t* __restrict__ ntask, uint32_t* __restrict__ hist) {
  ZKT_SIDE_PRIO;
  __shared__ uint32_t h[SIZE_BINS];
  for (int i = threadIdx.x; i < SIZE_BINS; i += 256) h[i] = 0;
  __syncthreads();
  size_t i = (size_t)blockIdx.x * 256 + threadIdx.x;
  if (i < m) {
    uint32_t c = counts[i], nt = ntasks_of(c, chunk);
    ntask[i] = nt;
    atomicAdd(&h[CHUNK - task_size_of(c, nt)], nt);
  }
  __syncthreads();
  for (int k = threadIdx.x; k < SIZE_BINS; k += 256) if (h[k]) atomicAdd(&hist[k], h[k]);
}
static constexpr uint32_t HOT_NT = 512, HOT_CAP = 64, HOT_FAN = 64;
static __global__ void __launch_bounds__(256) k_task_scatter(const uint32_t* __restrict__ counts, size_t m, uint32_t chunk, const uint32_t* __restrict__ size_hist,
                                                      uint32_t* __restrict__ bincur, uint2* __restrict__ order, uint32_t* __restrict__ hot) {
  ZKT_SIDE_PRIO;
  __shared__ uint32_t h[SIZE_BINS], base[SIZE_BINS], binoff[SIZE_BINS + 1], scan[256];
  __shared__ uint32_t hot_n, hot_b[256], hot_pos[256], hot_nt[256];
  for (int i = threadIdx.x; i < SIZE_BINS; i += 256) h[i] = 0;
  if (threadIdx.x == 0) hot_n = 0;
  {
    static_assert(SIZE_BINS <= 256, "one histogram bin per thread");
    uint32_t v = threadIdx.x < SIZE_BINS ? size_hist[threadIdx.x] : 0, tot;
    uint32_t ex = block_excl_scan_256(v, scan, tot);
    if (threadIdx.x < SIZE_BINS) binoff[threadIdx.x] = ex;
  }
  __syncthreads();
  size_t i = (size_t)blockIdx.x * 256 + threadIdx.x;
  uint32_t bin = 0, rank = 0, nt = 1;
  if (i < m) { uint32_t c = counts[i]; nt = ntasks_of(c, chunk); bin = CHUNK - task_size_of(c, nt); rank = atomicAdd(&h[bin], nt); }
  __syncthreads();
  for (int k = threadIdx.x; k < SIZE_BINS; k += 256) if (h[k]) base[k] = binoff[k] + atomicAdd(&bincur[k], h[k]);
  __syncthreads();
  if (i < m) {
    const uint32_t pos = base[bin] + rank;
    if (nt <= 16) { for (uint32_t k = 0; k < nt; ++k) order[pos + k] = make_uint2((uint32_t)i, k); }
    else { const uint32_t slot = atomicAdd(&hot_n, 1u); hot_b[slot] = (uint32_t)i; hot_pos[slot] = pos; hot_nt[slot] = nt; }
    if (nt > HOT_NT) { const uint32_t g = atomicAdd(&hot[0], 1u); if (g < HOT_CAP) hot[1 + g] = (uint32_t)i; }
  }
  __syncthreads();
  for (uint32_t hb = 0; hb < hot_n; ++hb) {
    const uint32_t b = hot_b[hb], pos = hot_pos[hb], cnt = hot_nt[hb];
    for (uint32_t k = threadIdx.x; k < cnt; k += 256) order[pos + k] = make_uint2(b, k);
  }
}

#ifndef ZKT_ACC_ATTR
#define ZKT_ACC_ATTR
#endif
template <class F>
__global__ void __launch_bounds__(64) ZKT_ACC_ATTR k_accumulate(const uint32_t* __restrict__ table, const uint32_t* __restrict__ entries,
                                                   const uint32_t* __restrict__ offsets, const uint2* __restrict__ order,
                                                   const uint32_t* __restrict__ task_off, size_t nbuckets,
                                                   uint32_t* __restrict__ sums, uint32_t* __restrict__ partial) {
  size_t t = (size_t)blockIdx.x * 64 + threadIdx.x;
  if (t >= task_off[nbuckets]) return;
  const uint2 tk = order[t];
  const size_t b = tk.x;
  const uint32_t t0 = task_off[b], nt = task_off[b + 1] - t0;
  const uint32_t off = offsets[b], cnt = offsets[b + 1] - off;
  uint32_t beg = off, end = off + cnt;
  if (nt != 1) {
    const uint32_t q = cnt / nt, r = cnt - q * nt;
    beg = off + tk.y * q + (tk.y < r ? tk.y : r); end = beg + q + (tk.y < r ? 1u : 0u);
  }
  constexpr int CW = Coord<F>::CW, XYW = 4 * CW;
  Xyzz<F> acc = xyzz_inf<F>();
  typedef typename F::E E;
  uint32_t ent = beg < end ? entries[beg] : 0, ent_next = beg + 1 < end ? entries[beg + 1] : 0;
  const uint32_t* p = table + (size_t)(ent & 0x7fffffffu) * (2 * CW);
#ifndef ZKT_ACC_PREFETCH_MAX_CW
#define ZKT_ACC_PREFETCH_MAX_CW 16
#endif
  if constexpr (CW <= ZKT_ACC_PREFETCH_MAX_CW) {
    E nx = Coord<F>::ld(p), ny = Coord<F>::ld(p + CW);
    for (uint32_t e = beg; e < end; ++e) {
      E x = nx, y = ny;
      const bool negate = ent >> 31;
      if (e + 1 < end) {
        ent = ent_next;
        ent_next = e + 2 < end ? entries[e + 2] : 0;
        p = table + (size_t)(ent & 0x7fffffffu) * (2 * CW);
        nx = Coord<F>::ld(p); ny = Coord<F>::ld(p + CW);
      }
      if (negate) y = F::neg(y);
      acc = xyzz_add_aff<F>(acc, x, y);
    }
  } else {
    for (uint32_t e = beg; e < end; ++e) {
      E x = Coord<F>::ld(p), y = Coord<F>::ld(p + CW);
      const bool negate = ent >> 31;
      ent = ent_next;
      ent_next = e + 2 < end ? entries[e + 2] : 0;
      p = table + (size_t)(ent & 0x7fffffffu) * (2 * CW);
      if (negate) y = F::neg(y);
      acc = xyzz_add_aff<F>(acc, x, y);
    }
  }
  st_xy<F>(nt == 1 ? sums + b * XYW : partial + (size_t)(t0 + tk.y) * XYW, acc);
}

}
#include "msm_reduce_coop.h"
namespace zkt {

template <class F>
__global__ void __launch_bounds__(64) k_join_windows(const uint32_t* __restrict__ win_jac, int nwin, int c, uint32_t* __restrict__ out_jac, uint32_t* __restrict__ out_abi) {
  ZKT_SIDE_PRIO;
  constexpr int CW = Coord<F>::CW, XYW = 4 * CW, JW = 3 * CW;
  __shared__ uint32_t lds[16 * JW];
  const int t = threadIdx.x;
  auto ldj = [](const uint32_t* p) { return Jac<F>{Coord<F>::ld(p), Coord<F>::ld(p + CW), Coord<F>::ld(p + 2 * CW)}; };
  auto stj = [](uint32_t* p, const Jac<F>& a) { Coord<F>::st(p, a.X); Coord<F>::st(p + CW, a.Y); Coord<F>::st(p + 2 * CW, a.Z); };
  Jac<F> v = jac_inf<F>();
  if (t < nwin) {
    v = ldj(win_jac + (size_t)t * XYW);
    for (int d = 0; d < c * t; ++d) v = jac_dbl(v);
  }
  for (int d = 16; d >= 1; d >>= 1) {
    if (t >= d && t < 2 * d) stj(lds + (t - d) * JW, v);
    __syncthreads();
    if (t < d) v = jac_add(v, ldj(lds + t * JW));
    __syncthreads();
  }
  if (t == 0) {
    stj(out_jac, v);
    if (out_abi) PtIO<F>::st(out_abi, jac_to_aff(v));
  }
}

namespace {
struct MsmWs {
  uint32_t *zero_begin, *counts, *cursor, *size_hist, *size_off, *size_cur, *hot, *zero_end;
  uint32_t *offsets, *entries, *slot, *sums, *colsum, *rowsum, *clsA, *clsB, *win_jac, *scan_tmp, *ntask, *task_off, *partial, *hot_part;
  uint32_t *tilehist, *tileoff, *blkoff, *subhist, *part_scan; uint2* rec;
  uint2* order; size_t max_tasks;
};
MsmWs carve(const MsmPlan& P, void* workspace) {
  const size_t B = P.nbuckets, XYW = 4 * (size_t)coord_words(P.grp);
  uint8_t* ws = (uint8_t*)workspace;
  MsmWs w;
  w.zero_begin = (uint32_t*)ws;
  w.counts = (uint32_t*)ws; ws += (B + 1) * 4;
  w.cursor = (uint32_t*)ws; ws += (B + 1) * 4;
  w.size_hist = (uint32_t*)ws; ws += (SIZE_BINS + 1) * 4;
  w.size_off = (uint32_t*)ws; ws += (SIZE_BINS + 1) * 4;
  w.size_cur = (uint32_t*)ws; ws += (SIZE_BINS + 1) * 4;
  w.hot = (uint32_t*)ws; ws += (HOT_CAP + 1) * 4;
  w.zero_end = (uint32_t*)ws;
  w.offsets = (uint32_t*)ws; ws += (B + 1) * 4;
  ws = (uint8_t*)(((uintptr_t)ws + 255) & ~(uintptr_t)255);
  w.entries = (uint32_t*)ws; ws += (size_t)P.nwin * P.n * 4;
  ws = (uint8_t*)(((uintptr_t)ws + 255) & ~(uintptr_t)255);
  w.slot = (uint32_t*)ws; ws += (size_t)P.nwin * P.n * 4;
  ws = (uint8_t*)(((uintptr_t)ws + 255) & ~(uintptr_t)255);
  w.sums = (uint32_t*)ws; ws += B * XYW * 4;
  const size_t nw = P.direct ? (size_t)P.nwin : 1;
  w.colsum = (uint32_t*)ws; ws += nw * 1024 * XYW * 4;
  w.rowsum = (uint32_t*)ws; ws += nw * 1024 * XYW * 4;
  w.clsA = (uint32_t*)ws; ws += nw * 32 * WB_SPLIT * XYW * 4;
  w.clsB = (uint32_t*)ws; ws += nw * 32 * WB_SPLIT * XYW * 4;
  w.win_jac = (uint32_t*)ws; ws += nw * XYW * 4;
  w.scan_tmp = (uint32_t*)ws; ws += 1024 * 4;
  w.ntask = (uint32_t*)ws; ws += (B + 1) * 4;
  w.task_off = (uint32_t*)ws; ws += (B + 1) * 4;
  w.max_tasks = B + (size_t)P.nwin * P.n / P.chunk + 1;
  ws = (uint8_t*)(((uintptr_t)ws + 255) & ~(uintptr_t)255);
  w.order = (uint2*)ws; ws += w.max_tasks * 8;
  w.partial = (uint32_t*)ws; ws += w.max_tasks * XYW * 4;
  w.hot_part = (uint32_t*)ws; ws += (size_t)HOT_CAP * HOT_FAN * XYW * 4;
  {
    const PartDims d = part_dims(P.n, P.nbuckets, P.nwin);
    ws = (uint8_t*)(((uintptr_t)ws + 255) & ~(uintptr_t)255);
    w.rec = (uint2*)ws; ws += (((size_t)P.nwin * P.n * 8) + 255) & ~(size_t)255;
    w.tilehist = (uint32_t*)ws; ws += ((size_t)d.P * d.ntiles + 1) * 4;
    w.tileoff = (uint32_t*)ws; ws += ((size_t)d.P * d.ntiles + 1) * 4;
    w.blkoff = (uint32_t*)ws; ws += ((size_t)d.P + 1) * 4;
    w.part_scan = (uint32_t*)ws; ws += ((size_t)d.P * d.ntiles / 2048 + 2) * 4;
    ws = (uint8_t*)(((uintptr_t)ws + 255) & ~(uintptr_t)255);
    w.subhist = (uint32_t*)ws; ws += (size_t)d.maxblk * PART_SUB * 4;
  }
  return w;
}
}

static __global__ void __launch_bounds__(256) k_zero_words(uint32_t* __restrict__ p, int head_words, size_t quads, int tail_words) {
  const size_t i = (size_t)blockIdx.x * 256 + threadIdx.x;
  if (i < (size_t)head_words) p[i] = 0u;
  uint4* q = reinterpret_cast<uint4*>(p + head_words);
  if (i < quads) q[i] = uint4{0u, 0u, 0u, 0u};
  if (i < (size_t)tail_words) p[(size_t)head_words + quads * 4 + i] = 0u;
}
static hipError_t zero_async(void* ptr, size_t bytes, hipStream_t s) {
  if (bytes == 0) return hipSuccess;
  if (((uintptr_t)ptr & 3u) || (bytes & 3u)) return hipErrorInvalidValue;
  size_t words = bytes / 4;
  int head = (int)(((16u - ((uintptr_t)ptr & 15u)) & 15u) / 4);
  if ((size_t)head > words) head = (int)words;
  words -= (size_t)head;
  const size_t quads = words / 4; const int tail = (int)(words % 4);
  size_t items = quads > (size_t)tail ? quads : (size_t)tail;
  if (items < (size_t)head) items = (size_t)head;
  hipLaunchKernelGGL(k_zero_words, dim3(grid_blocks(items)), dim3(256), 0, s, (uint32_t*)ptr, head, quads, tail);
  return hipGetLastError();
}
hipError_t PART(launch_msm_sort)(const MsmPlan& P, const uint8_t* inf, const uint32_t* scalars, void* workspace, hipStream_t s) {
  const size_t B = P.nbuckets, n = P.n;
  MsmWs w = carve(P, workspace);
  hipError_t e;
  if ((e = zero_async(w.zero_begin, (uint8_t*)w.zero_end - (uint8_t*)w.zero_begin, s)) != hipSuccess) return e;
  const PartDims pd = part_dims(n, B, P.nwin);
  const bool partition = (size_t)P.nwin * n >= (size_t(1) << 22);
  if (n && partition && pd.P <= PART_MAXP) {
    const uint32_t wb = P.direct ? (uint32_t)P.half : 0u;
    hipLaunchKernelGGL(k_part_tiles<false>, dim3(pd.ntiles), dim3(PART_TPB), 0, s, scalars, inf, n, P.c, P.nwin, wb, pd.P, pd.ntiles, w.tilehist, (const uint32_t*)nullptr, (uint2*)nullptr);
    launch_scan(w.tilehist, w.tileoff, (size_t)pd.P * pd.ntiles, w.part_scan, s);
    hipLaunchKernelGGL(k_part_tiles<true>, dim3(pd.ntiles), dim3(PART_TPB), 0, s, scalars, inf, n, P.c, P.nwin, wb, pd.P, pd.ntiles, (uint32_t*)nullptr, (const uint32_t*)w.tileoff, w.rec);
    hipLaunchKernelGGL(k_part_blocks, dim3(1), dim3(256), 0, s, (const uint32_t*)w.tileoff, pd.P, pd.ntiles, w.blkoff);
    hipLaunchKernelGGL(k_part_chunks<false>, dim3(pd.maxblk), dim3(256), 0, s, (const uint32_t*)w.tileoff, pd.P, pd.ntiles, (const uint32_t*)w.blkoff, (const uint2*)w.rec,
                       w.subhist, (const uint32_t*)nullptr, B, (uint32_t*)nullptr);
    hipLaunchKernelGGL(k_part_offsets, dim3(pd.P), dim3(PART_SUB), 0, s, (const uint32_t*)w.tileoff, pd.P, pd.ntiles, (const uint32_t*)w.blkoff, w.subhist, B, w.counts, w.offsets);
    hipLaunchKernelGGL(k_part_chunks<true>, dim3(pd.maxblk), dim3(256), 0, s, (const uint32_t*)w.tileoff, pd.P, pd.ntiles, (const uint32_t*)w.blkoff, (const uint2*)w.rec,
                       w.subhist, (const uint32_t*)w.offsets, B, w.entries);
  } else if (n) {
    const unsigned g = grid_blocks(n);
    const uint32_t wb = P.direct ? (uint32_t)P.half : 0u;
    hipLaunchKernelGGL(k_digits<false>, dim3(g), dim3(256), 0, s, scalars, inf, n, P.c, P.nwin, wb, w.counts, (const uint32_t*)nullptr, w.slot, (uint32_t*)nullptr);
    launch_scan(w.counts, w.offsets, B, w.scan_tmp, s);
    hipLaunchKernelGGL(k_digits<true>, dim3(g), dim3(256), 0, s, scalars, inf, n, P.c, P.nwin, wb, (uint32_t*)nullptr, (const uint32_t*)w.offsets, w.slot, w.entries);
  } else {
    if ((e = zero_async(w.offsets, (B + 1) * 4, s)) != hipSuccess) return e;
  }
  hipLaunchKernelGGL(k_task_count, dim3(grid_blocks(B)), dim3(256), 0, s, w.counts, B, P.chunk, w.ntask, w.size_hist);
  launch_scan(w.ntask, w.task_off, B, w.scan_tmp, s);
  hipLaunchKernelGGL(k_task_scatter, dim3(grid_blocks(B)), dim3(256), 0, s, w.counts, B, P.chunk, (const uint32_t*)w.size_hist, w.size_cur, w.order, w.hot);
  return hipGetLastError();
}
hipError_t PART(launch_msm_accumulate)(const MsmPlan& P, const uint32_t* table, void* workspace, hipStream_t s) {
  MsmWs w = carve(P, workspace);
#if defined(ZKT_MSM_PART_OTHER) && !defined(ZKT_G2_ONE_LANE)
  if (P.grp == G_G2)
    return ::zkt_launch_accumulate_g2_pair(table, (const uint32_t*)w.entries, (const uint32_t*)w.offsets, (const void*)w.order, (const uint32_t*)w.task_off, P.nbuckets,
                                           w.sums, w.partial, w.max_tasks, s);
#endif
  MSM_DISPATCH(P.grp, hipLaunchKernelGGL(k_accumulate<F>, dim3(grid_blocks(w.max_tasks, 64)), dim3(64), 0, s, table, (const uint32_t*)w.entries,
                                         (const uint32_t*)w.offsets, (const uint2*)w.order, (const uint32_t*)w.task_off, P.nbuckets, w.sums, w.partial));
  return hipGetLastError();
}
hipError_t PART(launch_msm_reduce)(const MsmPlan& P, void* workspace, uint32_t* dev_result_jac, uint32_t* dev_out_abi, hipStream_t s) {
  const size_t B = P.direct ? P.half : P.nbuckets;
  MsmWs w = carve(P, workspace);
  const size_t NLO = B < 1024 ? B : 1024, NHI = B / NLO;
  int lo_bits = 0; while ((size_t(1) << lo_bits) < NLO) ++lo_bits;
  int hi_bits = 0; while ((size_t(1) << hi_bits) < NHI) ++hi_bits;
  const int nbA = lo_bits + 1, nbB = NHI > 1 ? hi_bits : 0;
  int RS = 1;
  while (NHI > 1 && (size_t)(2 * RS) * NHI <= 1024 && NLO / (size_t)(2 * RS) >= 64 && NLO / (size_t)(2 * RS) >= NHI) RS *= 2;
  const size_t NROW = (size_t)RS * NHI;
  if (P.direct) {
    const unsigned ny = (unsigned)P.nwin;
    MSM_DISPATCH(P.grp,
      hipLaunchKernelGGL(k_merge_hot<F>, dim3(HOT_FAN, HOT_CAP), dim3(RED_TPB), 0, s, (const uint32_t*)w.task_off, (const uint32_t*)w.partial, (const uint32_t*)w.hot, w.hot_part);
      hipLaunchKernelGGL(k_merge_partials<F>, dim3((unsigned)((P.nbuckets + RED_NG - 1) / RED_NG < 4096 ? (P.nbuckets + RED_NG - 1) / RED_NG : 4096)), dim3(RED_TPB), 0, s, (const uint32_t*)w.task_off, P.nbuckets, (const uint32_t*)w.partial, (const uint32_t*)w.hot, (const uint32_t*)w.hot_part, w.sums);
      hipLaunchKernelGGL(k_marginals<F>, dim3((unsigned)(NLO + (NHI > 1 ? NROW : 0)), ny), dim3(RED_TPB), 0, s, (const uint32_t*)w.sums, NLO, NHI, RS, w.colsum, w.rowsum);
      hipLaunchKernelGGL(k_weight_bits<F>, dim3((unsigned)(nbA + nbB) * WB_SPLIT, ny), dim3(WB_TPB), 0, s, (const uint32_t*)w.colsum, NLO, nbA, (const uint32_t*)w.rowsum, NHI, RS, w.clsA, w.clsB);
      hipLaunchKernelGGL(k_combine<F>, dim3(1, ny), dim3(CMB_TPB), 0, s, (const uint32_t*)w.clsA, nbA, (const uint32_t*)w.clsB, nbB, lo_bits, w.win_jac, (uint32_t*)nullptr);
      hipLaunchKernelGGL(k_join_windows<F>, dim3(1), dim3(64), 0, s, (const uint32_t*)w.win_jac, P.nwin, P.c, dev_result_jac, dev_out_abi));
    return hipGetLastError();
  }
  MSM_DISPATCH(P.grp,
    hipLaunchKernelGGL(k_merge_hot<F>, dim3(HOT_FAN, HOT_CAP), dim3(RED_TPB), 0, s, (const uint32_t*)w.task_off, (const uint32_t*)w.partial, (const uint32_t*)w.hot, w.hot_part);
    hipLaunchKernelGGL(k_merge_partials<F>, dim3((unsigned)((B + RED_NG - 1) / RED_NG < 4096 ? (B + RED_NG - 1) / RED_NG : 4096)), dim3(RED_TPB), 0, s, (const uint32_t*)w.task_off, B, (const uint32_t*)w.partial, (const uint32_t*)w.hot, (const uint32_t*)w.hot_part, w.sums);
    hipLaunchKernelGGL(k_marginals<F>, dim3((unsigned)(NLO + (NHI > 1 ? NROW : 0))), dim3(RED_TPB), 0, s, (const uint32_t*)w.sums, NLO, NHI, RS, w.colsum, w.rowsum);
    hipLaunchKernelGGL(k_weight_bits<F>, dim3((unsigned)(nbA + nbB) * WB_SPLIT), dim3(WB_TPB), 0, s, (const uint32_t*)w.colsum, NLO, nbA, (const uint32_t*)w.rowsum, NHI, RS, w.clsA, w.clsB);
    hipLaunchKernelGGL(k_combine<F>, dim3(1), dim3(CMB_TPB), 0, s, (const uint32_t*)w.clsA, nbA, (const uint32_t*)w.clsB, nbB, lo_bits, dev_result_jac, dev_out_abi));
  return hipGetLastError();
}

hipError_t PART(launch_msm_precompute)(int grp, uint32_t* table, uint8_t* inf, size_t n, int c, int nwin, uint32_t* tmp, hipStream_t s) {
  if (n == 0) return hipSuccess;
  MSM_DISPATCH(grp, hipLaunchKernelGGL(k_precompute<F>, dim3(grid_blocks(n, 64)), dim3(64), 0, s, table, inf, n, c, nwin, tmp));
  return hipGetLastError();
}

template <class F>
__global__ void __launch_bounds__(64) k_jac_sum_to_affine(const uint32_t* __restrict__ parts, size_t count, size_t stride, uint32_t* __restrict__ out_abi) {
  constexpr int CW = Coord<F>::CW, JW = 3 * CW;
  __shared__ uint32_t lds[32 * JW];
  const int t = threadIdx.x;
  auto ldj = [](const uint32_t* p) { return Jac<F>{Coord<F>::ld(p), Coord<F>::ld(p + CW), Coord<F>::ld(p + 2 * CW)}; };
  auto stj = [](uint32_t* p, const Jac<F>& a) { Coord<F>::st(p, a.X); Coord<F>::st(p + CW, a.Y); Coord<F>::st(p + 2 * CW, a.Z); };
  Jac<F> v = jac_inf<F>();
  for (size_t i = t; i < count; i += 64) v = jac_add<F>(v, ldj(parts + i * stride));
  for (int d = 32; d >= 1; d >>= 1) {
    if (t >= d && t < 2 * d) stj(lds + (t - d) * JW, v);
    __syncthreads();
    if (t < d && (size_t)(t + d) < count) v = jac_add<F>(v, ldj(lds + t * JW));
    __syncthreads();
  }
  if (t == 0) PtIO<F>::st(out_abi, jac_to_aff(v));
}
template <class F>
__global__ void __launch_bounds__(64) k_jac_add(const uint32_t* __restrict__ a, const uint32_t* __restrict__ b, uint32_t* __restrict__ out) {
  if (threadIdx.x) return;
  constexpr int CW = Coord<F>::CW;
  const Jac<F> x{Coord<F>::ld(a), Coord<F>::ld(a + CW), Coord<F>::ld(a + 2 * CW)}, y{Coord<F>::ld(b), Coord<F>::ld(b + CW), Coord<F>::ld(b + 2 * CW)};
  const Jac<F> r = jac_add<F>(x, y);
  Coord<F>::st(out, r.X); Coord<F>::st(out + CW, r.Y); Coord<F>::st(out + 2 * CW, r.Z);
}
hipError_t PART(launch_msm_jac_add)(int grp, const uint32_t* a, const uint32_t* b, uint32_t* out, hipStream_t s) {
  MSM_DISPATCH(grp, hipLaunchKernelGGL(k_jac_add<F>, dim3(1), dim3(64), 0, s, a, b, out));
  return hipGetLastError();
}
hipError_t PART(launch_msm_jac_sum_to_affine)(int grp, const uint32_t* parts, size_t count, size_t stride, uint32_t* out_abi, hipStream_t s) {
  MSM_DISPATCH(grp, hipLaunchKernelGGL(k_jac_sum_to_affine<F>, dim3(1), dim3(64), 0, s, parts, count, stride, out_abi));
  return hipGetLastError();
}


#if defined(ZKT_MSM_PART_G1)
#define ZKT_MSM_FWD(SUF) \
  hipError_t launch_msm_to_kernel_layout##SUF(int, const uint32_t*, uint32_t*, uint8_t*, size_t, hipStream_t); \
  hipError_t launch_msm_precompute##SUF(int, uint32_t*, uint8_t*, size_t, int, int, uint32_t*, hipStream_t); \
  hipError_t launch_msm_sort##SUF(const MsmPlan&, const uint8_t*, const uint32_t*, void*, hipStream_t); \
  hipError_t launch_msm_accumulate##SUF(const MsmPlan&, const uint32_t*, void*, hipStream_t); \
  hipError_t launch_msm_reduce##SUF(const MsmPlan&, void*, uint32_t*, uint32_t*, hipStream_t); \
  hipError_t launch_msm_jac_add##SUF(int, const uint32_t*, const uint32_t*, uint32_t*, hipStream_t); \
  hipError_t launch_msm_jac_sum_to_affine##SUF(int, const uint32_t*, size_t, size_t, uint32_t*, hipStream_t);
ZKT_MSM_FWD(_other) ZKT_MSM_FWD(_secp)
#define ZKT_MSM_BY_GROUP(grp, NAME, ...) ((grp) == G_G1 ? NAME##_g1(__VA_ARGS__) : (grp) == G_SECP ? NAME##_secp(__VA_ARGS__) : NAME##_other(__VA_ARGS__))
hipError_t launch_msm_to_kernel_layout(int grp, const uint32_t* a, uint32_t* t, uint8_t* i, size_t n, hipStream_t s) { return ZKT_MSM_BY_GROUP(grp, launch_msm_to_kernel_layout, grp, a, t, i, n, s); }
hipError_t launch_msm_precompute(int grp, uint32_t* t, uint8_t* i, size_t n, int c, int nw, uint32_t* tmp, hipStream_t s) { return ZKT_MSM_BY_GROUP(grp, launch_msm_precompute, grp, t, i, n, c, nw, tmp, s); }
hipError_t launch_msm_sort(const MsmPlan& P, const uint8_t* i, const uint32_t* k, void* w, hipStream_t s) { return ZKT_MSM_BY_GROUP(P.grp, launch_msm_sort, P, i, k, w, s); }
hipError_t launch_msm_accumulate(const MsmPlan& P, const uint32_t* t, void* w, hipStream_t s) { return ZKT_MSM_BY_GROUP(P.grp, launch_msm_accumulate, P, t, w, s); }
hipError_t launch_msm_reduce(const MsmPlan& P, void* w, uint32_t* j, uint32_t* o, hipStream_t s) { return ZKT_MSM_BY_GROUP(P.grp, launch_msm_reduce, P, w, j, o, s); }
hipError_t launch_msm_jac_add(int grp, const uint32_t* a, const uint32_t* b, uint32_t* o, hipStream_t s) { return ZKT_MSM_BY_GROUP(grp, launch_msm_jac_add, grp, a, b, o, s); }
hipError_t launch_msm_jac_sum_to_affine(int grp, const uint32_t* p, size_t c, size_t st, uint32_t* o, hipStream_t s) { return ZKT_MSM_BY_GROUP(grp, launch_msm_jac_sum_to_affine, grp, p, c, st, o, s); }
#endif

}
```

Before: 422.4 million.

## Split MSM workspace into sort and bucket rings shared across slots

Splits the MSM workspace into a sort part and a bucket part. For large inputs, per-slot workspaces are replaced by small rings of sort and bucket buffers reused across submissions, guarded by free events so pipelined MSMs can overlap. The sort buffer is released once the partial merge finishes, before the final reduction completes. Per-slot result buffers are also pooled into one allocation. The aim is a smaller memory footprint and better cache/TLB behaviour, at the cost of extra cross-stream event waits that could serialize submissions.

```diff
diff --git a/zk-toolkit_amd/csrc/zkt_api.cpp b/zk-toolkit_amd/csrc/zkt_api.cpp
--- a/zk-toolkit_amd/csrc/zkt_api.cpp
+++ b/zk-toolkit_amd/csrc/zkt_api.cpp
@@ -140,6 +140,19 @@
 }
 
 static constexpr int MSM_SLOTS = 8;
+#ifndef ZKT_MSM_RING_SORT
+#define ZKT_MSM_RING_SORT 2
+#endif
+#ifndef ZKT_MSM_RING_BUCKET
+#define ZKT_MSM_RING_BUCKET 3
+#endif
+static constexpr int MSM_RING_SORT = ZKT_MSM_RING_SORT, MSM_RING_BUCKET = ZKT_MSM_RING_BUCKET;
+static constexpr size_t MSM_RING_MIN_N = size_t(1) << 19;
+struct MsmRingPart {
+  void* ws = nullptr;
+  hipEvent_t e_free = nullptr;
+  bool used = false;
+};
 struct MsmSlot {
   hipEvent_t e_in = nullptr, e_sorted = nullptr, e_acc0 = nullptr, e_acc1 = nullptr, e_done = nullptr;
   void* workspace = nullptr;
@@ -161,6 +174,9 @@
   hipStream_t s_sort = nullptr, s_acc = nullptr, s_tail[NTAIL] = {};
   bool own_streams = true, acc_owned = false, grouped = false; int tail_base = 0, tail_span = 0;
   MsmSlot slot[MSM_SLOTS];
+  uint8_t* d_results = nullptr; uint8_t* h_results = nullptr;
+  MsmRingPart ring_sort[MSM_RING_SORT], ring_bucket[MSM_RING_BUCKET];
+  uint64_t submitted = 0;
   std::mutex mu;
 };
 struct zkt_g1_bases : zkt_bases_impl {};
@@ -178,17 +194,34 @@
 }
 static bool debug_poison() { static const bool on = [] { const char* e = getenv("ZKT_DEBUG_POISON"); return e && *e == '1'; }(); return on; }
 static bool msm_graphs() { static const bool on = [] { const char* e = getenv("ZKT_MSM_GRAPH"); return !(e && *e == '0'); }(); return on; }
+static int slots_create(zkt_bases_impl* h) {
+  const size_t jb = padded(3 * grp_coord_bytes(h->grp)), ob = padded(abi_pt_bytes(h->grp));
+  HIPCHK(hipMalloc((void**)&h->d_results, MSM_SLOTS * (jb + ob)));
+  HIPCHK(hipHostMalloc((void**)&h->h_results, MSM_SLOTS * ob, hipHostMallocDefault));
+  for (int k = 0; k < MSM_SLOTS; ++k) {
+    MsmSlot& S = h->slot[k];
+    HIPCHK(hipEventCreateWithFlags(&S.e_in, hipEventDisableTiming)); HIPCHK(hipEventCreateWithFlags(&S.e_sorted, hipEventDisableTiming));
+    HIPCHK(hipEventCreate(&S.e_acc0)); HIPCHK(hipEventCreate(&S.e_acc1)); HIPCHK(hipEventCreateWithFlags(&S.e_done, hipEventDisableTiming));
+    S.d_result_jac = (uint32_t*)(h->d_results + k * (jb + ob));
+    S.d_out_abi = (uint32_t*)(h->d_results + k * (jb + ob) + jb);
+    S.h_out = h->h_results + k * ob;
+  }
+  if (h->n < MSM_RING_MIN_N) return ZKT_OK;
+  for (MsmRingPart& R : h->ring_sort) { HIPCHK(hipMalloc(&R.ws, h->plan.ws_sort_bytes)); HIPCHK(hipEventCreateWithFlags(&R.e_free, hipEventDisableTiming)); }
+  for (MsmRingPart& R : h->ring_bucket) { HIPCHK(hipMalloc(&R.ws, h->plan.ws_bucket_bytes)); HIPCHK(hipEventCreateWithFlags(&R.e_free, hipEventDisableTiming)); }
+  if (debug_poison()) {
+    for (MsmRingPart& R : h->ring_sort) HIPCHK(hipMemset(R.ws, 0xA5, h->plan.ws_sort_bytes));
+    for (MsmRingPart& R : h->ring_bucket) HIPCHK(hipMemset(R.ws, 0xA5, h->plan.ws_bucket_bytes));
+    HIPCHK(hipDeviceSynchronize());
+  }
+  return ZKT_OK;
+}
 static int slot_ready(zkt_bases_impl* h, int k) {
   int rc = streams_ready(h); if (rc) return rc;
   MsmSlot& S = h->slot[k];
-  if (S.workspace) return ZKT_OK;
-  HIPCHK(hipEventCreateWithFlags(&S.e_in, hipEventDisableTiming)); HIPCHK(hipEventCreateWithFlags(&S.e_sorted, hipEventDisableTiming));
-  HIPCHK(hipEventCreate(&S.e_acc0)); HIPCHK(hipEventCreate(&S.e_acc1)); HIPCHK(hipEventCreateWithFlags(&S.e_done, hipEventDisableTiming));
+  if (S.workspace || h->n >= MSM_RING_MIN_N) return ZKT_OK;
   HIPCHK(hipMalloc(&S.workspace, h->plan.ws_bytes));
   if (debug_poison()) { HIPCHK(hipMemset(S.workspace, 0xA5, h->plan.ws_bytes)); HIPCHK(hipDeviceSynchronize()); }
-  HIPCHK(hipMalloc((void**)&S.d_result_jac, 3 * grp_coord_bytes(h->grp)));
-  HIPCHK(hipMalloc((void**)&S.d_out_abi, abi_pt_bytes(h->grp)));
-  HIPCHK(hipHostMalloc((void**)&S.h_out, abi_pt_bytes(h->grp), hipHostMallocDefault));
   return ZKT_OK;
 }
 
@@ -486,9 +519,15 @@
   for (MsmSlot& S : h->slot) {
     for (hipEvent_t ev : {S.e_in, S.e_sorted, S.e_acc0, S.e_acc1, S.e_done}) if (ev) hipEventDestroy(ev);
     for (hipGraphExec_t& ge : S.gexec) if (ge) { (void)hipGraphExecDestroy(ge); ge = nullptr; }
-    if (S.workspace) hipFree(S.workspace); if (S.d_result_jac) hipFree(S.d_result_jac); if (S.d_out_abi) hipFree(S.d_out_abi);
-    if (S.h_out) hipHostFree(S.h_out);
-  }
+    if (S.workspace) hipFree(S.workspace);
+  }
+  for (MsmRingPart* ring : {h->ring_sort, h->ring_bucket})
+    for (int k = 0; k < (ring == h->ring_sort ? MSM_RING_SORT : MSM_RING_BUCKET); ++k) {
+      if (ring[k].e_free) hipEventDestroy(ring[k].e_free);
+      if (ring[k].ws) hipFree(ring[k].ws);
+    }
+  if (h->d_results) hipFree(h->d_results);
+  if (h->h_results) hipHostFree(h->h_results);
   delete h;
 }
 static int bases_from_device(int grp, const void* dev_bases, size_t n, void* stream, zkt_bases_impl** out) {
@@ -496,6 +535,7 @@
   if (!out || (n && !dev_bases) || n >= (size_t(1) << 26)) return ZKT_ERR_SHAPE;
   zkt_bases_impl* h = new zkt_bases_impl(); h->n = n; h->grp = grp;
   int rc = bases_build(h, (const uint32_t*)dev_bases, (hipStream_t)stream);
+  if (!rc) rc = slots_create(h);
   if (rc) { bases_free(h); return rc; }
   *out = h; return ZKT_OK;
 }
@@ -512,7 +552,7 @@
 }
 static hipStream_t slot_tail_stream(zkt_bases_impl* h, int slot) {
   if (h->grouped) return h->s_tail[(h->tail_base + slot % h->tail_span) % zkt_bases_impl::GROUP_TAILS];
-  const bool small = h->n < (size_t(1) << 19);
+  const bool small = h->n < MSM_RING_MIN_N;
   return h->s_tail[small ? slot % zkt_bases_impl::NTAIL : slot % 2];
 }
 static int msm_submit_locked(zkt_bases_impl* h, const uint64_t* dev_scalars, size_t n, void* stream, int slot) {
@@ -521,7 +561,7 @@
   int rc = slot_ready(h, slot); if (rc) return rc;
   MsmSlot& S = h->slot[slot];
   HIPCHK(hipEventRecord(S.e_in, (hipStream_t)stream));
-  const bool small = h->n < (size_t(1) << 19);
+  const bool small = h->n < MSM_RING_MIN_N;
   hipStream_t st = slot_tail_stream(h, slot);
   hipStream_t ss = small ? st : h->s_sort;
   HIPCHK(hipStreamWaitEvent(ss, S.e_in, 0));
@@ -533,9 +573,10 @@
       if (S.gexec[hit]) { (void)hipGraphExecDestroy(S.gexec[hit]); S.gexec[hit] = nullptr; }
       hipGraph_t graph = nullptr;
       HIPCHK(hipStreamBeginCapture(st, hipStreamCaptureModeRelaxed));
+      void* wb = (uint8_t*)S.workspace + h->plan.ws_sort_bytes;
       hipError_t e = launch_msm_sort(h->plan, h->inf, (const uint32_t*)dev_scalars, S.workspace, st);
-      if (e == hipSuccess) e = launch_msm_accumulate(h->plan, h->table, S.workspace, st);
-      if (e == hipSuccess) e = launch_msm_reduce(h->plan, S.workspace, S.d_result_jac, S.d_out_abi, st);
+      if (e == hipSuccess) e = launch_msm_accumulate(h->plan, h->table, S.workspace, wb, st);
+      if (e == hipSuccess) e = launch_msm_reduce(h->plan, S.workspace, wb, S.d_result_jac, S.d_out_abi, st);
       const hipError_t e2 = hipStreamEndCapture(st, &graph);
       if (e != hipSuccess || e2 != hipSuccess || !graph) { if (graph) (void)hipGraphDestroy(graph); HIPCHK(e != hipSuccess ? e : (e2 != hipSuccess ? e2 : hipErrorUnknown)); }
       e = hipGraphInstantiate(&S.gexec[hit], graph, nullptr, nullptr, 0);
@@ -550,15 +591,24 @@
     return ZKT_OK;
   }
   S.timed = true;
-  HIPCHK(launch_msm_sort(h->plan, h->inf, (const uint32_t*)dev_scalars, S.workspace, ss));
+  MsmRingPart* RS = small ? nullptr : &h->ring_sort[h->submitted % MSM_RING_SORT];
+  MsmRingPart* RB = small ? nullptr : &h->ring_bucket[h->submitted % MSM_RING_BUCKET];
+  void* ws = small ? S.workspace : RS->ws;
+  void* wb = small ? (uint8_t*)S.workspace + h->plan.ws_sort_bytes : RB->ws;
+  if (!small) ++h->submitted;
+  if (RS && RS->used) HIPCHK(hipStreamWaitEvent(ss, RS->e_free, 0));
+  HIPCHK(launch_msm_sort(h->plan, h->inf, (const uint32_t*)dev_scalars, ws, ss));
   HIPCHK(hipEventRecord(S.e_sorted, ss));
   hipStream_t sa = small ? st : h->s_acc;
   HIPCHK(hipStreamWaitEvent(sa, S.e_sorted, 0));
+  if (RB && RB->used) HIPCHK(hipStreamWaitEvent(sa, RB->e_free, 0));
   HIPCHK(hipEventRecord(S.e_acc0, sa));
-  HIPCHK(launch_msm_accumulate(h->plan, h->table, S.workspace, sa));
+  HIPCHK(launch_msm_accumulate(h->plan, h->table, ws, wb, sa));
   HIPCHK(hipEventRecord(S.e_acc1, sa));
   HIPCHK(hipStreamWaitEvent(st, S.e_acc1, 0));
-  HIPCHK(launch_msm_reduce(h->plan, S.workspace, S.d_result_jac, S.d_out_abi, st));
+  HIPCHK(launch_msm_reduce(h->plan, ws, wb, S.d_result_jac, S.d_out_abi, st, RS ? RS->e_free : nullptr));
+  if (RS) RS->used = true;
+  if (RB) { HIPCHK(hipEventRecord(RB->e_free, st)); RB->used = true; }
   HIPCHK(hipMemcpyAsync(S.h_out, S.d_out_abi, abi_pt_bytes(h->grp), hipMemcpyDeviceToHost, st));
   HIPCHK(hipEventRecord(S.e_done, st));
   S.busy = true;
@@ -644,7 +694,7 @@
   const size_t ptb = abi_pt_bytes(grp), cb = grp_coord_bytes(grp);
   uint8_t* blob = nullptr;
   const size_t o_abi = 0, o_sc = padded(n * ptb), o_tab = o_sc + padded(n * 32), o_inf = o_tab + padded(n * 2 * cb), o_jac = o_inf + padded(n),
-               o_out = o_jac + padded(4 * cb), o_ws = o_out + padded(ptb), total = o_ws + plan.ws_bytes;
+               o_out = o_jac + padded(4 * cb), o_ws = o_out + padded(ptb), o_wb = o_ws + plan.ws_sort_bytes, total = o_ws + plan.ws_bytes;
   HIPCHK(hipMalloc((void**)&blob, total));
   if (debug_poison()) { HIPCHK(hipMemset(blob, 0xA5, total)); HIPCHK(hipDeviceSynchronize()); }
   std::lock_guard<std::mutex> lk(g.mu);
@@ -654,8 +704,8 @@
   if (!fail(hipMemcpyAsync(blob + o_abi, bases, n * ptb, hipMemcpyHostToDevice, s)) && !fail(hipMemcpyAsync(blob + o_sc, scalars, n * 32, hipMemcpyHostToDevice, s)) &&
       !fail(launch_msm_to_kernel_layout(grp, (const uint32_t*)(blob + o_abi), (uint32_t*)(blob + o_tab), blob + o_inf, n, s)) &&
       !fail(launch_msm_sort(plan, blob + o_inf, (const uint32_t*)(blob + o_sc), blob + o_ws, s)) &&
-      !fail(launch_msm_accumulate(plan, (const uint32_t*)(blob + o_tab), blob + o_ws, s)) &&
-      !fail(launch_msm_reduce(plan, blob + o_ws, (uint32_t*)(blob + o_jac), (uint32_t*)(blob + o_out), s)) &&
+      !fail(launch_msm_accumulate(plan, (const uint32_t*)(blob + o_tab), blob + o_ws, blob + o_wb, s)) &&
+      !fail(launch_msm_reduce(plan, blob + o_ws, blob + o_wb, (uint32_t*)(blob + o_jac), (uint32_t*)(blob + o_out), s)) &&
       !fail(hipMemcpyAsync(out, blob + o_out, ptb, hipMemcpyDeviceToHost, s)))
     fail(hipStreamSynchronize(s));
   else hipStreamSynchronize(s);
diff --git a/zk-toolkit_amd/csrc/zkt_internal.h b/zk-toolkit_amd/csrc/zkt_internal.h
--- a/zk-toolkit_amd/csrc/zkt_internal.h
+++ b/zk-toolkit_amd/csrc/zkt_internal.h
@@ -87,6 +87,8 @@
   int nwin;
   size_t nbuckets;
   size_t ws_bytes;
+  size_t ws_sort_bytes;
+  size_t ws_bucket_bytes;
   int direct;
   size_t half;
   uint32_t chunk;
@@ -95,9 +97,10 @@
 MsmPlan msm_plan_direct(size_t n, int grp);
 hipError_t launch_msm_to_kernel_layout(int grp, const uint32_t* abi_pts, uint32_t* table, uint8_t* base_inf, size_t n, hipStream_t s);
 hipError_t launch_msm_precompute(int grp, uint32_t* table, uint8_t* inf, size_t n, int c, int nwin, uint32_t* tmp, hipStream_t s);
-hipError_t launch_msm_sort(const MsmPlan& plan, const uint8_t* base_inf, const uint32_t* scalars, void* workspace, hipStream_t s);
-hipError_t launch_msm_accumulate(const MsmPlan& plan, const uint32_t* table, void* workspace, hipStream_t s);
-hipError_t launch_msm_reduce(const MsmPlan& plan, void* workspace, uint32_t* dev_result_jac, uint32_t* dev_out_abi, hipStream_t s);
+hipError_t launch_msm_sort(const MsmPlan& plan, const uint8_t* base_inf, const uint32_t* scalars, void* ws_sort, hipStream_t s);
+hipError_t launch_msm_accumulate(const MsmPlan& plan, const uint32_t* table, const void* ws_sort, void* ws_bucket, hipStream_t s);
+hipError_t launch_msm_reduce(const MsmPlan& plan, const void* ws_sort, void* ws_bucket, uint32_t* dev_result_jac, uint32_t* dev_out_abi, hipStream_t s,
+                             hipEvent_t sort_read = nullptr);
 hipError_t launch_msm_jac_add(int grp, const uint32_t* a, const uint32_t* b, uint32_t* out, hipStream_t s);
 hipError_t launch_msm_jac_sum_to_affine(int grp, const uint32_t* jac_partials, size_t count, size_t stride_words, uint32_t* out_abi_pt, hipStream_t s);
 
diff --git a/zk-toolkit_amd/csrc/zkt_msm.hip b/zk-toolkit_amd/csrc/zkt_msm.hip
--- a/zk-toolkit_amd/csrc/zkt_msm.hip
+++ b/zk-toolkit_amd/csrc/zkt_msm.hip
@@ -41,6 +41,7 @@
 #if defined(ZKT_MSM_PART_G1)
 static constexpr uint32_t MSM_CHUNK_MAX = 128;
 static uint32_t pick_chunk(size_t entries, int grp);
+static void msm_plan_split(MsmPlan& p);
 MsmPlan msm_plan(size_t n, int grp) {
   MsmPlan p; p.n = n; p.grp = grp;
   const size_t XYW = 4 * (size_t)coord_words(grp);
@@ -65,6 +66,7 @@
   b += 4096;
   p.ws_bytes = b;
   p.direct = 0; p.half = p.nbuckets;
+  msm_plan_split(p);
   return p;
 }
 static uint32_t pick_chunk(size_t entries, int grp) {
@@ -93,6 +95,7 @@
   b += part_ws_bytes(n, p.nbuckets, p.nwin);
   b += 8192;
   p.ws_bytes = b;
+  msm_plan_split(p);
   return p;
 }
 #endif
@@ -514,14 +517,14 @@
 namespace {
 struct MsmWs {
   uint32_t *zero_begin, *counts, *cursor, *size_hist, *size_off, *size_cur, *hot, *zero_end;
-  uint32_t *offsets, *entries, *slot, *sums, *colsum, *rowsum, *clsA, *clsB, *win_jac, *scan_tmp, *ntask, *task_off, *partial, *hot_part;
+  uint32_t *offsets, *entries, *slot, *scan_tmp, *ntask, *task_off;
   uint32_t *tilehist, *tileoff, *blkoff, *subhist, *part_scan; uint2* rec;
   uint2* order; size_t max_tasks;
+  uint32_t *sums, *colsum, *rowsum, *clsA, *clsB, *win_jac, *partial, *hot_part;
 };
-MsmWs carve(const MsmPlan& P, void* workspace) {
-  const size_t B = P.nbuckets, XYW = 4 * (size_t)coord_words(P.grp);
-  uint8_t* ws = (uint8_t*)workspace;
-  MsmWs w;
+inline uint8_t* align256(uint8_t* p) { return (uint8_t*)(((uintptr_t)p + 255) & ~(uintptr_t)255); }
+uint8_t* carve_sort(const MsmPlan& P, MsmWs& w, uint8_t* ws) {
+  const size_t B = P.nbuckets;
   w.zero_begin = (uint32_t*)ws;
   w.counts = (uint32_t*)ws; ws += (B + 1) * 4;
   w.cursor = (uint32_t*)ws; ws += (B + 1) * 4;
@@ -531,11 +534,30 @@
   w.hot = (uint32_t*)ws; ws += (HOT_CAP + 1) * 4;
   w.zero_end = (uint32_t*)ws;
   w.offsets = (uint32_t*)ws; ws += (B + 1) * 4;
-  ws = (uint8_t*)(((uintptr_t)ws + 255) & ~(uintptr_t)255);
+  ws = align256(ws);
   w.entries = (uint32_t*)ws; ws += (size_t)P.nwin * P.n * 4;
-  ws = (uint8_t*)(((uintptr_t)ws + 255) & ~(uintptr_t)255);
+  ws = align256(ws);
   w.slot = (uint32_t*)ws; ws += (size_t)P.nwin * P.n * 4;
-  ws = (uint8_t*)(((uintptr_t)ws + 255) & ~(uintptr_t)255);
+  w.scan_tmp = (uint32_t*)ws; ws += 1024 * 4;
+  w.ntask = (uint32_t*)ws; ws += (B + 1) * 4;
+  w.task_off = (uint32_t*)ws; ws += (B + 1) * 4;
+  w.max_tasks = B + (size_t)P.nwin * P.n / P.chunk + 1;
+  ws = align256(ws);
+  w.order = (uint2*)ws; ws += w.max_tasks * 8;
+  const PartDims d = part_dims(P.n, P.nbuckets, P.nwin);
+  ws = align256(ws);
+  w.rec = (uint2*)ws; ws += (((size_t)P.nwin * P.n * 8) + 255) & ~(size_t)255;
+  w.tilehist = (uint32_t*)ws; ws += ((size_t)d.P * d.ntiles + 1) * 4;
+  w.tileoff = (uint32_t*)ws; ws += ((size_t)d.P * d.ntiles + 1) * 4;
+  w.blkoff = (uint32_t*)ws; ws += ((size_t)d.P + 1) * 4;
+  w.part_scan = (uint32_t*)ws; ws += ((size_t)d.P * d.ntiles / 2048 + 2) * 4;
+  ws = align256(ws);
+  w.subhist = (uint32_t*)ws; ws += (size_t)d.maxblk * PART_SUB * 4;
+  return ws;
+}
+uint8_t* carve_bucket(const MsmPlan& P, MsmWs& w, uint8_t* ws) {
+  const size_t B = P.nbuckets, XYW = 4 * (size_t)coord_words(P.grp);
+  const size_t max_tasks = B + (size_t)P.nwin * P.n / P.chunk + 1;
   w.sums = (uint32_t*)ws; ws += B * XYW * 4;
   const size_t nw = P.direct ? (size_t)P.nwin : 1;
   w.colsum = (uint32_t*)ws; ws += nw * 1024 * XYW * 4;
@@ -543,28 +565,27 @@
   w.clsA = (uint32_t*)ws; ws += nw * 32 * WB_SPLIT * XYW * 4;
   w.clsB = (uint32_t*)ws; ws += nw * 32 * WB_SPLIT * XYW * 4;
   w.win_jac = (uint32_t*)ws; ws += nw * XYW * 4;
-  w.scan_tmp = (uint32_t*)ws; ws += 1024 * 4;
-  w.ntask = (uint32_t*)ws; ws += (B + 1) * 4;
-  w.task_off = (uint32_t*)ws; ws += (B + 1) * 4;
-  w.max_tasks = B + (size_t)P.nwin * P.n / P.chunk + 1;
-  ws = (uint8_t*)(((uintptr_t)ws + 255) & ~(uintptr_t)255);
-  w.order = (uint2*)ws; ws += w.max_tasks * 8;
-  w.partial = (uint32_t*)ws; ws += w.max_tasks * XYW * 4;
+  ws = align256(ws);
+  w.partial = (uint32_t*)ws; ws += max_tasks * XYW * 4;
   w.hot_part = (uint32_t*)ws; ws += (size_t)HOT_CAP * HOT_FAN * XYW * 4;
-  {
-    const PartDims d = part_dims(P.n, P.nbuckets, P.nwin);
-    ws = (uint8_t*)(((uintptr_t)ws + 255) & ~(uintptr_t)255);
-    w.rec = (uint2*)ws; ws += (((size_t)P.nwin * P.n * 8) + 255) & ~(size_t)255;
-    w.tilehist = (uint32_t*)ws; ws += ((size_t)d.P * d.ntiles + 1) * 4;
-    w.tileoff = (uint32_t*)ws; ws += ((size_t)d.P * d.ntiles + 1) * 4;
-    w.blkoff = (uint32_t*)ws; ws += ((size_t)d.P + 1) * 4;
-    w.part_scan = (uint32_t*)ws; ws += ((size_t)d.P * d.ntiles / 2048 + 2) * 4;
-    ws = (uint8_t*)(((uintptr_t)ws + 255) & ~(uintptr_t)255);
-    w.subhist = (uint32_t*)ws; ws += (size_t)d.maxblk * PART_SUB * 4;
-  }
+  return ws;
+}
+MsmWs carve(const MsmPlan& P, const void* ws_sort, const void* ws_bucket) {
+  MsmWs w{};
+  carve_sort(P, w, (uint8_t*)ws_sort);
+  if (ws_bucket) carve_bucket(P, w, (uint8_t*)ws_bucket);
   return w;
 }
 }
+#if defined(ZKT_MSM_PART_G1)
+static void msm_plan_split(MsmPlan& p) {
+  MsmWs w{};
+  uint8_t* const base = (uint8_t*)(uintptr_t)4096;
+  p.ws_sort_bytes = ((size_t)(carve_sort(p, w, base) - base) + 1024 + 255) & ~(size_t)255;
+  p.ws_bucket_bytes = ((size_t)(carve_bucket(p, w, base) - base) + 1024 + 255) & ~(size_t)255;
+  if (p.ws_sort_bytes + p.ws_bucket_bytes > p.ws_bytes) p.ws_bytes = p.ws_sort_bytes + p.ws_bucket_bytes;
+}
+#endif
 
 static __global__ void __launch_bounds__(256) k_zero_words(uint32_t* __restrict__ p, int head_words, size_t quads, int tail_words) {
   const size_t i = (size_t)blockIdx.x * 256 + threadIdx.x;
@@ -586,9 +607,9 @@
   hipLaunchKernelGGL(k_zero_words, dim3(grid_blocks(items)), dim3(256), 0, s, (uint32_t*)ptr, head, quads, tail);
   return hipGetLastError();
 }
-hipError_t PART(launch_msm_sort)(const MsmPlan& P, const uint8_t* inf, const uint32_t* scalars, void* workspace, hipStream_t s) {
+hipError_t PART(launch_msm_sort)(const MsmPlan& P, const uint8_t* inf, const uint32_t* scalars, void* ws_sort, hipStream_t s) {
   const size_t B = P.nbuckets, n = P.n;
-  MsmWs w = carve(P, workspace);
+  MsmWs w = carve(P, ws_sort, nullptr);
   hipError_t e;
   if ((e = zero_async(w.zero_begin, (uint8_t*)w.zero_end - (uint8_t*)w.zero_begin, s)) != hipSuccess) return e;
   const PartDims pd = part_dims(n, B, P.nwin);
@@ -618,8 +639,8 @@
   hipLaunchKernelGGL(k_task_scatter, dim3(grid_blocks(B)), dim3(256), 0, s, w.counts, B, P.chunk, (const uint32_t*)w.size_hist, w.size_cur, w.order, w.hot);
   return hipGetLastError();
 }
-hipError_t PART(launch_msm_accumulate)(const MsmPlan& P, const uint32_t* table, void* workspace, hipStream_t s) {
-  MsmWs w = carve(P, workspace);
+hipError_t PART(launch_msm_accumulate)(const MsmPlan& P, const uint32_t* table, const void* ws_sort, void* ws_bucket, hipStream_t s) {
+  MsmWs w = carve(P, ws_sort, ws_bucket);
 #if defined(ZKT_MSM_PART_OTHER) && !defined(ZKT_G2_ONE_LANE)
   if (P.grp == G_G2)
     return ::zkt_launch_accumulate_g2_pair(table, (const uint32_t*)w.entries, (const uint32_t*)w.offsets, (const void*)w.order, (const uint32_t*)w.task_off, P.nbuckets,
@@ -629,9 +650,10 @@
                                          (const uint32_t*)w.offsets, (const uint2*)w.order, (const uint32_t*)w.task_off, P.nbuckets, w.sums, w.partial));
   return hipGetLastError();
 }
-hipError_t PART(launch_msm_reduce)(const MsmPlan& P, void* workspace, uint32_t* dev_result_jac, uint32_t* dev_out_abi, hipStream_t s) {
+hipError_t PART(launch_msm_reduce)(const MsmPlan& P, const void* ws_sort, void* ws_bucket, uint32_t* dev_result_jac, uint32_t* dev_out_abi, hipStream_t s,
+                                   hipEvent_t sort_read) {
   const size_t B = P.direct ? P.half : P.nbuckets;
-  MsmWs w = carve(P, workspace);
+  MsmWs w = carve(P, ws_sort, ws_bucket);
   const size_t NLO = B < 1024 ? B : 1024, NHI = B / NLO;
   int lo_bits = 0; while ((size_t(1) << lo_bits) < NLO) ++lo_bits;
   int hi_bits = 0; while ((size_t(1) << hi_bits) < NHI) ++hi_bits;
@@ -644,6 +666,7 @@
     MSM_DISPATCH(P.grp,
       hipLaunchKernelGGL(k_merge_hot<F>, dim3(HOT_FAN, HOT_CAP), dim3(RED_TPB), 0, s, (const uint32_t*)w.task_off, (const uint32_t*)w.partial, (const uint32_t*)w.hot, w.hot_part);
       hipLaunchKernelGGL(k_merge_partials<F>, dim3((unsigned)((P.nbuckets + RED_NG - 1) / RED_NG < 4096 ? (P.nbuckets + RED_NG - 1) / RED_NG : 4096)), dim3(RED_TPB), 0, s, (const uint32_t*)w.task_off, P.nbuckets, (const uint32_t*)w.partial, (const uint32_t*)w.hot, (const uint32_t*)w.hot_part, w.sums);
+      if (sort_read) (void)hipEventRecord(sort_read, s);
       hipLaunchKernelGGL(k_marginals<F>, dim3((unsigned)(NLO + (NHI > 1 ? NROW : 0)), ny), dim3(RED_TPB), 0, s, (const uint32_t*)w.sums, NLO, NHI, RS, w.colsum, w.rowsum);
       hipLaunchKernelGGL(k_weight_bits<F>, dim3((unsigned)(nbA + nbB) * WB_SPLIT, ny), dim3(WB_TPB), 0, s, (const uint32_t*)w.colsum, NLO, nbA, (const uint32_t*)w.rowsum, NHI, RS, w.clsA, w.clsB);
       hipLaunchKernelGGL(k_combine<F>, dim3(1, ny), dim3(CMB_TPB), 0, s, (const uint32_t*)w.clsA, nbA, (const uint32_t*)w.clsB, nbB, lo_bits, w.win_jac, (uint32_t*)nullptr);
@@ -653,6 +676,7 @@
   MSM_DISPATCH(P.grp,
     hipLaunchKernelGGL(k_merge_hot<F>, dim3(HOT_FAN, HOT_CAP), dim3(RED_TPB), 0, s, (const uint32_t*)w.task_off, (const uint32_t*)w.partial, (const uint32_t*)w.hot, w.hot_part);
     hipLaunchKernelGGL(k_merge_partials<F>, dim3((unsigned)((B + RED_NG - 1) / RED_NG < 4096 ? (B + RED_NG - 1) / RED_NG : 4096)), dim3(RED_TPB), 0, s, (const uint32_t*)w.task_off, B, (const uint32_t*)w.partial, (const uint32_t*)w.hot, (const uint32_t*)w.hot_part, w.sums);
+    if (sort_read) (void)hipEventRecord(sort_read, s);
     hipLaunchKernelGGL(k_marginals<F>, dim3((unsigned)(NLO + (NHI > 1 ? NROW : 0))), dim3(RED_TPB), 0, s, (const uint32_t*)w.sums, NLO, NHI, RS, w.colsum, w.rowsum);
     hipLaunchKernelGGL(k_weight_bits<F>, dim3((unsigned)(nbA + nbB) * WB_SPLIT), dim3(WB_TPB), 0, s, (const uint32_t*)w.colsum, NLO, nbA, (const uint32_t*)w.rowsum, NHI, RS, w.clsA, w.clsB);
     hipLaunchKernelGGL(k_combine<F>, dim3(1), dim3(CMB_TPB), 0, s, (const uint32_t*)w.clsA, nbA, (const uint32_t*)w.clsB, nbB, lo_bits, dev_result_jac, dev_out_abi));
@@ -705,8 +729,8 @@
   hipError_t launch_msm_to_kernel_layout##SUF(int, const uint32_t*, uint32_t*, uint8_t*, size_t, hipStream_t); \
   hipError_t launch_msm_precompute##SUF(int, uint32_t*, uint8_t*, size_t, int, int, uint32_t*, hipStream_t); \
   hipError_t launch_msm_sort##SUF(const MsmPlan&, const uint8_t*, const uint32_t*, void*, hipStream_t); \
-  hipError_t launch_msm_accumulate##SUF(const MsmPlan&, const uint32_t*, void*, hipStream_t); \
-  hipError_t launch_msm_reduce##SUF(const MsmPlan&, void*, uint32_t*, uint32_t*, hipStream_t); \
+  hipError_t launch_msm_accumulate##SUF(const MsmPlan&, const uint32_t*, const void*, void*, hipStream_t); \
+  hipError_t launch_msm_reduce##SUF(const MsmPlan&, const void*, void*, uint32_t*, uint32_t*, hipStream_t, hipEvent_t); \
   hipError_t launch_msm_jac_add##SUF(int, const uint32_t*, const uint32_t*, uint32_t*, hipStream_t); \
   hipError_t launch_msm_jac_sum_to_affine##SUF(int, const uint32_t*, size_t, size_t, uint32_t*, hipStream_t);
 ZKT_MSM_FWD(_other) ZKT_MSM_FWD(_secp)
@@ -714,8 +738,8 @@
 hipError_t launch_msm_to_kernel_layout(int grp, const uint32_t* a, uint32_t* t, uint8_t* i, size_t n, hipStream_t s) { return ZKT_MSM_BY_GROUP(grp, launch_msm_to_kernel_layout, grp, a, t, i, n, s); }
 hipError_t launch_msm_precompute(int grp, uint32_t* t, uint8_t* i, size_t n, int c, int nw, uint32_t* tmp, hipStream_t s) { return ZKT_MSM_BY_GROUP(grp, launch_msm_precompute, grp, t, i, n, c, nw, tmp, s); }
 hipError_t launch_msm_sort(const MsmPlan& P, const uint8_t* i, const uint32_t* k, void* w, hipStream_t s) { return ZKT_MSM_BY_GROUP(P.grp, launch_msm_sort, P, i, k, w, s); }
-hipError_t launch_msm_accumulate(const MsmPlan& P, const uint32_t* t, void* w, hipStream_t s) { return ZKT_MSM_BY_GROUP(P.grp, launch_msm_accumulate, P, t, w, s); }
-hipError_t launch_msm_reduce(const MsmPlan& P, void* w, uint32_t* j, uint32_t* o, hipStream_t s) { return ZKT_MSM_BY_GROUP(P.grp, launch_msm_reduce, P, w, j, o, s); }
+hipError_t launch_msm_accumulate(const MsmPlan& P, const uint32_t* t, const void* ws, void* wb, hipStream_t s) { return ZKT_MSM_BY_GROUP(P.grp, launch_msm_accumulate, P, t, ws, wb, s); }
+hipError_t launch_msm_reduce(const MsmPlan& P, const void* ws, void* wb, uint32_t* j, uint32_t* o, hipStream_t s, hipEvent_t e) { return ZKT_MSM_BY_GROUP(P.grp, launch_msm_reduce, P, ws, wb, j, o, s, e); }
 hipError_t launch_msm_jac_add(int grp, const uint32_t* a, const uint32_t* b, uint32_t* o, hipStream_t s) { return ZKT_MSM_BY_GROUP(grp, launch_msm_jac_add, grp, a, b, o, s); }
 hipError_t launch_msm_jac_sum_to_affine(int grp, const uint32_t* p, size_t c, size_t st, uint32_t* o, hipStream_t s) { return ZKT_MSM_BY_GROUP(grp, launch_msm_jac_sum_to_affine, grp, p, c, st, o, s); }
 #endif
```

Result: faster. 427.8 million (median of 6 runs) (+1.3%).
